# yangdongchao/RSTnet

Measured on NVIDIA H100. Metric: codec_frames_per_s, higher is better.
Workload: dtype f32

## Files before the change

### include/rstnet_b200.h

```cpp
#ifndef RSTNET_B200_H
#define RSTNET_B200_H

#include <stdint.h>

#ifdef __cplusplus
extern "C" {
#endif

typedef void* rstnet_stream_t;

enum { RSTNET_ACT_NONE = 0, RSTNET_ACT_ELU = 1, RSTNET_ACT_GELU = 2 };

int rstnet_version(void);
const char* rstnet_last_error(void);
int64_t rstnet_launch_count(void);
uint32_t rstnet_device_error_flags(int clear);

typedef struct {
  const float* A;
  int64_t a_batch_stride, a_row_stride;
  const float* Wt;
  const float* bias;
  const float* scale;
  const float* R;
  int64_t r_batch_stride, r_row_stride;
  float* C;
  int64_t c_batch_stride, c_row_stride;
  int32_t batch, rows, N, K;
  int32_t pre_act, post_act;
  int32_t taps;
  int64_t tap_stride;
} rstnet_gemm_rows_args;
int rstnet_gemm_rows_f32(const rstnet_gemm_rows_args* args, rstnet_stream_t stream);

typedef struct rstnet_tc_plan rstnet_tc_plan;
typedef struct {
  const float* A;
  int64_t a_i_stride, a_o_stride;
  int32_t a_c_extent, a_i_extent, a_o_extent;
  int32_t taps, tap_di, tap_do, o_mul;
  const float* W;
  const float* W_lo;
  int32_t N, Kc;
  int32_t I_out, O_out;
  float* C;
  int64_t c_i_stride, c_o_stride, c_split_stride;
  const float* R;
  int64_t r_i_stride, r_o_stride, r_split_stride;
  const float* bias;
  const float* scale;
  int32_t n_split;
  int32_t pre_act, post_act, precision;
  float* C2;
  int32_t act2;
} rstnet_tc_gemm_desc;
int rstnet_tc_gemm_create(const rstnet_tc_gemm_desc* desc, rstnet_tc_plan** out);
int rstnet_tc_gemm_run(const rstnet_tc_plan* plan, rstnet_stream_t stream);
void rstnet_tc_gemm_destroy(rstnet_tc_plan* plan);
int rstnet_tc_gemm_grid(const rstnet_tc_plan* plan, int32_t* grid_x, int32_t* grid_y, int32_t* tile_n);
int rstnet_tc_gemm_create_ex(const rstnet_tc_gemm_desc* desc, int32_t kpair, rstnet_tc_plan** out);
int rstnet_tc_gemm_kpair(const rstnet_tc_plan* plan, int32_t* on);
typedef struct rstnet_tc_resblock_plan rstnet_tc_resblock_plan;
typedef struct {
  const float* Y;
  int64_t y_i_stride, y_o_stride;
  int32_t channels;
  int32_t I_out, O_out, y_rows;
  const float* W1;
  const float* W1_lo;
  const float* b1;
  const float* W2;
  const float* W2_lo;
  const float* b2;
  float* out;
  int64_t out_i_stride, out_o_stride;
} rstnet_tc_resblock_desc;
int rstnet_tc_resblock_create(const rstnet_tc_resblock_desc* desc, rstnet_tc_resblock_plan** out);
int rstnet_tc_resblock_run(const rstnet_tc_resblock_plan* plan, rstnet_stream_t stream);
void rstnet_tc_resblock_destroy(rstnet_tc_resblock_plan* plan);

int rstnet_tf32_split_f32(const float* x, float* hi, float* lo, int64_t n, rstnet_stream_t stream);

int rstnet_conv1d_cin1_f32(const float* x, int64_t x_batch_stride, int64_t x_time_stride, const float* w, const float* bias,
                           float* out, float* out2 , int64_t out_batch_stride,
                           int64_t out_time_stride, int32_t batch, int32_t T, int32_t Cout, int32_t k,
                           int32_t post_act, int32_t act2, rstnet_stream_t stream);

int rstnet_conv1d_cout1_f32(const float* x, int64_t x_batch_stride, int64_t x_time_stride, const float* w,
                            const float* bias, float* out, int64_t out_batch_stride, int32_t batch,
                            int32_t T, int32_t Cin, int32_t k, rstnet_stream_t stream);

int rstnet_convtr1d_depthwise_f32(const float* x, int64_t x_batch_stride, int64_t x_time_stride,
                                  const float* w, float* out, int64_t out_batch_stride,
                                  int64_t out_time_stride, int32_t batch, int32_t T, int32_t C,
                                  int32_t stride, rstnet_stream_t stream);

int rstnet_rows_fill_f32(float* buf, int64_t batch_stride, int32_t batch, int32_t C, int32_t row0,
                         int32_t nrows, int32_t mode, int32_t src_row, const int64_t* only_if_zero,
                         int32_t only_if_zero_stride ,
                         int32_t channels_per_stream, rstnet_stream_t stream);
int rstnet_rows_fill_tail_f32(float* buf, int64_t batch_stride, int32_t batch, int32_t C, int32_t row0, int32_t nrows,
                              int32_t mode, const int64_t* valid, int64_t valid_div, int32_t channels_per_stream,
                              rstnet_stream_t stream);
typedef struct {
  float* buf;
  int64_t batch_stride;
  int32_t C, src_row, dst_row, nrows;
  int32_t cps;
  int32_t reserved;
} rstnet_row_copy;
int rstnet_rows_copy_table_f32(const rstnet_row_copy* table_dev, int32_t n_entries, int32_t batch,
                               const int64_t* active, rstnet_stream_t stream);
int rstnet_counter_add(int64_t* counter, int64_t delta, int32_t n, const int64_t* active ,
                       rstnet_stream_t stream);
int rstnet_counter_add_rows(int64_t* counter, const int64_t* delta, int32_t n, rstnet_stream_t stream);

int rstnet_layer_norm_f32(const float* x, int64_t x_batch_stride, const float* weight, const float* bias,
                          float* y, int32_t batch, int32_t rows_per_batch, int32_t dim, float eps,
                          rstnet_stream_t stream);

int rstnet_rope_kv_append_f32(float* qkv, int64_t q_batch_stride, int64_t q_time_stride, float* kv,
                              const int64_t* offset, int32_t offset_stride, const float* freqs, int32_t batch,
                              int32_t T, int32_t H, int32_t D, int32_t cap, rstnet_stream_t stream);
int rstnet_ring_attention_f32(const float* qkv, int64_t q_batch_stride, int64_t q_time_stride,
                              const float* kv, const int64_t* offset, int32_t offset_stride, float* out,
                              int64_t o_batch_stride, int64_t o_time_stride, int32_t batch, int32_t T,
                              int32_t H, int32_t D, int32_t cap, int32_t context, int32_t linear,
                              rstnet_stream_t stream);
int rstnet_rope_ring_attention_f32(const float* qkv, int64_t q_batch_stride, int64_t q_time_stride, float* kv,
                                   const int64_t* offset, int32_t offset_stride, const float* freqs, float* out,
                                   int64_t o_batch_stride, int64_t o_time_stride, int32_t batch, int32_t T, int32_t H,
                                   int32_t D, int32_t cap, int32_t context, rstnet_stream_t stream);

int64_t rstnet_rvq_encode_workspace(int64_t N, int32_t n_q, int32_t dim, int32_t bins);
int rstnet_rvq_encode_f32(const float* x, int64_t ldx, const float* E, const float* Et,
                          const float* enorm, int64_t* codes, void* work, int64_t N, int32_t T,
                          int32_t n_q, int32_t n_q_semantic, int32_t dim, int32_t bins,
                          int32_t time_major, rstnet_stream_t stream);
int rstnet_rvq_decode_gather_f32(const int64_t* codes, const float* E, float* q, int64_t N, int32_t T,
                                 int32_t n_q, int32_t n_q_semantic, int32_t dim, int32_t bins,
                                 int32_t time_major, rstnet_stream_t stream);

#define RSTNET_RESAMPLE_MAX_TABLE_BYTES (48 * 1024)
int rstnet_resample_f32(const float* x, int64_t x_row_stride, int64_t x_len, int64_t x_shift, const float* taps,
                        const int32_t* start, int32_t n, int32_t o, int32_t S, int32_t start_max, float* out,
                        int64_t out_row_stride, int64_t out_len, int32_t rows, rstnet_stream_t stream);

#define RSTNET_STFT_FRAMES_PER_BLOCK 16
int64_t rstnet_stft_loss_workspace(int32_t clips, int64_t max_len, int32_t hop);
int rstnet_stft_loss_sums_f32(const float* ref, const float* deg, const int64_t* offsets, const int64_t* lengths,
                              int32_t clips, int64_t min_len, int64_t max_len, int32_t n_fft, int32_t hop, int32_t win,
                              const float* twiddle, const float* window, double* sums, int32_t n_res, int32_t res,
                              void* ws, int64_t ws_bytes, rstnet_stream_t stream);

#define RSTNET_SISNR_SAMPLES_PER_BLOCK 8192
int64_t rstnet_sisnr_moments_workspace(int32_t clips, int64_t max_len);
int rstnet_sisnr_moments_f32(const float* ref, const float* deg, const int64_t* offsets, const int64_t* lengths,
                             int32_t clips, int64_t max_len, double* moments, void* ws, int64_t ws_bytes,
                             rstnet_stream_t stream);


typedef struct rstnet_skinny_plan rstnet_skinny_plan;
int64_t rstnet_skinny_gemm_workspace(int32_t M, int32_t N, int32_t max_splits);
int rstnet_skinny_gemm_create(const void* X, const void* W, const void* R, void* out, float* partial_ws,
                              int32_t M, int32_t N, int32_t K, int32_t max_splits, rstnet_skinny_plan** plan);
int rstnet_skinny_gemm_create_fused(const void* X, const void* W, const void* R, void* out, float* partial_ws,
                                    int32_t M, int32_t N, int32_t K, int32_t max_splits, int32_t fin_mode,
                                    const void* norm_w, void* aux_out, float eps, int32_t kyutai,
                                    rstnet_skinny_plan** plan);
int rstnet_skinny_gemm_run(const rstnet_skinny_plan* plan, rstnet_stream_t stream);
void rstnet_skinny_gemm_destroy(rstnet_skinny_plan* plan);

int rstnet_lm_embed_sum_bf16(const int64_t* seq, int32_t seq_stride, const void* wte, int64_t wte_rows,
                             const void* const* tables_dev, int64_t table_rows, int32_t n_q, int32_t E, void* x, int32_t rows,
                             rstnet_stream_t stream);
int rstnet_lm_embed_rows_bf16(const int64_t* ids, int32_t id_stride, const void* table, int64_t table_rows, int32_t D,
                              void* out, int32_t rows, rstnet_stream_t stream);
int rstnet_lm_rms_norm_bf16(const void* x, const void* w, void* y, int32_t rows, int32_t dim, float eps, int32_t kyutai,
                            rstnet_stream_t stream);
int rstnet_lm_rope_kv_append_bf16(const void* qkv, const void* cos_tab, const void* sin_tab, int64_t rope_rows, int32_t rope_n,
                                  const int64_t* offset, int32_t offset_stride ,
                                  const int32_t* row_stream, const int32_t* row_tl, void* q_out, void* kv, int32_t rows,
                                  int32_t B, int32_t n_head, int32_t n_kv, int32_t hs, int32_t cap, rstnet_stream_t stream);
#define RSTNET_KV_LOG2_PAGE_MIN 4
#define RSTNET_KV_LOG2_PAGE_MAX 12
int rstnet_lm_rope_kv_append_paged_bf16(const void* qkv, const void* cos_tab, const void* sin_tab, int64_t rope_rows,
                                        int32_t rope_n, const int64_t* offset, int32_t offset_stride, const int32_t* row_stream,
                                        const int32_t* row_tl, void* q_out, void* kv, int32_t rows, int32_t B, int32_t n_head,
                                        int32_t n_kv, int32_t hs, int32_t cap, const int32_t* page_table, int32_t pages_stride,
                                        int32_t log2_page, rstnet_stream_t stream);
int rstnet_lm_rope_pair_kv_append_bf16(const void* qkv, const int64_t* offset, int32_t offset_stride, void* q_out, void* kv,
                                       int32_t rows, int32_t B, int32_t H, int32_t hd, int32_t cap, const float* freqs,
                                       rstnet_stream_t stream);
int rstnet_lm_rope_pair_kv_append_paged_bf16(const void* qkv, const int64_t* offset, int32_t offset_stride, void* q_out, void* kv,
                                             int32_t rows, int32_t B, int32_t H, int32_t hd, int32_t cap, const float* freqs,
                                             const int32_t* page_table, int32_t pages_stride, int32_t log2_page,
                                             rstnet_stream_t stream);
int rstnet_lm_rope_pair_kv_append_rows_bf16(const void* qkv, const int64_t* offset, const int32_t* row_stream, const int32_t* row_tl,
                                            void* q_out, void* kv, int32_t rows, int32_t B, int32_t H, int32_t hd, int32_t cap,
                                            const float* freqs, rstnet_stream_t stream);
int rstnet_lm_ring_decode_attention_bf16(const void* q, const void* kv, const int64_t* offset, int32_t offset_stride,
                                         const int32_t* row_stream, const int32_t* row_tl, void* out, int32_t rows, int32_t B,
                                         int32_t n_head, int32_t n_kv, int32_t hs, int32_t cap, int32_t context,
                                         rstnet_stream_t stream);
int rstnet_lm_paged_decode_attention_bf16(const void* q, const void* kv, const int64_t* offset, int32_t offset_stride,
                                          const int32_t* row_stream, const int32_t* row_tl, void* out, int32_t rows, int32_t B,
                                          int32_t n_head, int32_t n_kv, int32_t hs, int32_t cap, int32_t context,
                                          const int32_t* page_table, int32_t pages_stride, int32_t log2_page,
                                          rstnet_stream_t stream);
int rstnet_lm_silu_mul_bf16(const void* ab, void* out, int32_t M, int32_t I, rstnet_stream_t stream);
int rstnet_lm_depth_attention_bf16(const void* qkv, void* kvd, void* out, int32_t B, int32_t H, int32_t hd, int32_t cap,
                                   int32_t step, int32_t ring_quirk, rstnet_stream_t stream);
int rstnet_lm_sample_params_bf16(const void* logits, int32_t rows, int32_t V, int32_t n_valid, const int32_t* n_valid_rows,
                                 int32_t n_valid_stride, int32_t top_k, float temp, float top_p, const int32_t* top_k_rows,
                                 const float* temp_rows, const float* top_p_rows, int32_t param_stride, uint32_t seed,
                                 const int64_t* step_counter, const int64_t* step_rows, const uint32_t* key_rows,
                                 int64_t* tokens, int32_t tok_stride, rstnet_stream_t stream);

int rstnet_lm_cross_entropy_bf16(const void* logits, int64_t row_stride, int32_t rows, int32_t V, int32_t groups,
                                 const int64_t* labels, const int64_t* ignore_ids, const float* weights,
                                 const int32_t* row_slot, int32_t n_slots, float* nll, int32_t* pred, double* acc,
                                 rstnet_stream_t stream);

int rstnet_lm_delay_cache_in(int64_t* cache, const int64_t* off, const int64_t* active, const int64_t* delays,
                             const int64_t* user, int32_t user_stride, int64_t* seq, int32_t seq_stride, int32_t B, int32_t K,
                             int32_t dep_q, int32_t CT, int64_t text_init, int64_t audio_init, rstnet_stream_t stream);
int rstnet_lm_delay_cache_out(int64_t* cache, int64_t* off, const int64_t* active, const int64_t* delays,
                              const int64_t* tokens, int32_t tok_stride, int64_t* out, int32_t out_stride, int64_t* valid,
                              int32_t B, int32_t K, int32_t dep_q, int32_t CT, int32_t max_delay, rstnet_stream_t stream);

typedef struct {
  void* base;
  int64_t stride_bytes;
  int64_t bytes;
  int32_t count;
  int64_t staging_offset;
} rstnet_segment;
int rstnet_segments_gather(const rstnet_segment* table_dev, int32_t n, void* staging, int32_t ctas, rstnet_stream_t s);
int rstnet_segments_scatter(const rstnet_segment* table_dev, int32_t n, const void* staging, int32_t ctas, rstnet_stream_t s);

#define RSTNET_KV_COPY_MAX_POOLS 256
int rstnet_kv_pages_copy(const void* const* pools, int32_t n_pools, const int32_t* pairs, int32_t n_pairs, int64_t page_bytes,
                         int32_t ctas, rstnet_stream_t s);

#define RSTNET_GEN_REC 5
enum { RSTNET_GEN_HELD = 0, RSTNET_GEN_FIXED = 1, RSTNET_GEN_WINDOWED = 2, RSTNET_GEN_ARGMAX = 4 };
enum { RSTNET_GEN_RUNNING = 0, RSTNET_GEN_LAST = 1, RSTNET_GEN_STOPPED = 2, RSTNET_GEN_IDLE = 3 };
int rstnet_lm_gen_rows_advance(const int64_t* tokens, int32_t tok_stride, int32_t* rec, int32_t* row_valid, int32_t valid_stride,
                               int32_t* status, int32_t B, int32_t dep_q, int32_t card, rstnet_stream_t stream);

#ifdef __cplusplus
}
#endif
#endif
```

### rstnet_b200/_lib.py

```python
from __future__ import annotations

import ctypes as C
import os

_HERE = os.path.dirname(os.path.abspath(__file__))
LIB_PATH = os.path.join(_HERE, "lib", "librstnet_b200.so")

ACT_NONE, ACT_ELU, ACT_GELU = 0, 1, 2

SYMBOLS = [
    "rstnet_version", "rstnet_last_error", "rstnet_launch_count", "rstnet_device_error_flags",
    "rstnet_gemm_rows_f32", "rstnet_tc_gemm_create", "rstnet_tc_gemm_run", "rstnet_tc_gemm_destroy", "rstnet_tc_gemm_grid",
    "rstnet_tc_gemm_create_ex", "rstnet_tc_gemm_kpair",
    "rstnet_tc_resblock_create", "rstnet_tc_resblock_run", "rstnet_tc_resblock_destroy", "rstnet_tf32_split_f32", "rstnet_conv1d_cin1_f32", "rstnet_conv1d_cout1_f32",
    "rstnet_convtr1d_depthwise_f32", "rstnet_rows_fill_f32", "rstnet_rows_copy_table_f32",
    "rstnet_counter_add", "rstnet_layer_norm_f32", "rstnet_rope_kv_append_f32",
    "rstnet_ring_attention_f32", "rstnet_rope_ring_attention_f32", "rstnet_rvq_encode_workspace", "rstnet_rvq_encode_f32",
    "rstnet_rvq_decode_gather_f32",
    "rstnet_skinny_gemm_workspace", "rstnet_skinny_gemm_create", "rstnet_skinny_gemm_create_fused", "rstnet_skinny_gemm_run", "rstnet_skinny_gemm_destroy",
    "rstnet_lm_embed_sum_bf16", "rstnet_lm_embed_rows_bf16", "rstnet_lm_rms_norm_bf16", "rstnet_lm_rope_kv_append_bf16",
    "rstnet_lm_rope_pair_kv_append_bf16",
    "rstnet_lm_ring_decode_attention_bf16", "rstnet_lm_silu_mul_bf16", "rstnet_lm_depth_attention_bf16",
    "rstnet_resample_f32", "rstnet_lm_delay_cache_in", "rstnet_lm_delay_cache_out", "rstnet_counter_add_rows",
    "rstnet_lm_cross_entropy_bf16", "rstnet_rows_fill_tail_f32", "rstnet_lm_sample_params_bf16",
    "rstnet_lm_rope_kv_append_paged_bf16", "rstnet_lm_paged_decode_attention_bf16", "rstnet_lm_rope_pair_kv_append_paged_bf16",
    "rstnet_stft_loss_workspace", "rstnet_stft_loss_sums_f32", "rstnet_sisnr_moments_workspace", "rstnet_sisnr_moments_f32",
    "rstnet_segments_gather", "rstnet_segments_scatter", "rstnet_lm_rope_pair_kv_append_rows_bf16",
    "rstnet_kv_pages_copy", "rstnet_lm_gen_rows_advance",
]

KV_LOG2_PAGE_MIN, KV_LOG2_PAGE_MAX = 4, 12
KV_COPY_MAX_POOLS = 256
GEN_REC = 5
GEN_HELD, GEN_FIXED, GEN_WINDOWED, GEN_ARGMAX = 0, 1, 2, 4
GEN_RUNNING, GEN_LAST, GEN_STOPPED, GEN_IDLE = 0, 1, 2, 3

RESAMPLE_MAX_TABLE_BYTES = 48 * 1024

STFT_FRAMES_PER_BLOCK = 16
SISNR_SAMPLES_PER_BLOCK = 8192


class GemmRowsArgs(C.Structure):
    _fields_ = [
        ("A", C.c_void_p), ("a_batch_stride", C.c_int64), ("a_row_stride", C.c_int64),
        ("Wt", C.c_void_p), ("bias", C.c_void_p), ("scale", C.c_void_p),
        ("R", C.c_void_p), ("r_batch_stride", C.c_int64), ("r_row_stride", C.c_int64),
        ("C", C.c_void_p), ("c_batch_stride", C.c_int64), ("c_row_stride", C.c_int64),
        ("batch", C.c_int32), ("rows", C.c_int32), ("N", C.c_int32), ("K", C.c_int32),
        ("pre_act", C.c_int32), ("post_act", C.c_int32), ("taps", C.c_int32), ("tap_stride", C.c_int64),
    ]


class TcGemmDesc(C.Structure):
    _fields_ = [
        ("A", C.c_void_p), ("a_i_stride", C.c_int64), ("a_o_stride", C.c_int64),
        ("a_c_extent", C.c_int32), ("a_i_extent", C.c_int32), ("a_o_extent", C.c_int32),
        ("taps", C.c_int32), ("tap_di", C.c_int32), ("tap_do", C.c_int32), ("o_mul", C.c_int32),
        ("W", C.c_void_p), ("W_lo", C.c_void_p), ("N", C.c_int32), ("Kc", C.c_int32), ("I_out", C.c_int32), ("O_out", C.c_int32),
        ("C", C.c_void_p), ("c_i_stride", C.c_int64), ("c_o_stride", C.c_int64), ("c_split_stride", C.c_int64),
        ("R", C.c_void_p), ("r_i_stride", C.c_int64), ("r_o_stride", C.c_int64), ("r_split_stride", C.c_int64),
        ("bias", C.c_void_p), ("scale", C.c_void_p),
        ("n_split", C.c_int32), ("pre_act", C.c_int32), ("post_act", C.c_int32), ("precision", C.c_int32),
        ("C2", C.c_void_p), ("act2", C.c_int32),
    ]


class TcResblockDesc(C.Structure):
    _fields_ = [
        ("Y", C.c_void_p), ("y_i_stride", C.c_int64), ("y_o_stride", C.c_int64),
        ("channels", C.c_int32), ("I_out", C.c_int32), ("O_out", C.c_int32), ("y_rows", C.c_int32),
        ("W1", C.c_void_p), ("W1_lo", C.c_void_p), ("b1", C.c_void_p),
        ("W2", C.c_void_p), ("W2_lo", C.c_void_p), ("b2", C.c_void_p),
        ("out", C.c_void_p), ("out_i_stride", C.c_int64), ("out_o_stride", C.c_int64),
    ]


class RowCopy(C.Structure):
    _fields_ = [("buf", C.c_void_p), ("batch_stride", C.c_int64), ("C", C.c_int32), ("src_row", C.c_int32),
                ("dst_row", C.c_int32), ("nrows", C.c_int32), ("cps", C.c_int32), ("reserved", C.c_int32)]


class Segment(C.Structure):
    _fields_ = [("base", C.c_void_p), ("stride_bytes", C.c_int64), ("bytes", C.c_int64), ("count", C.c_int32),
                ("staging_offset", C.c_int64)]


class RstnetError(RuntimeError):
    pass


_lib = None


def lib() -> C.CDLL:
    global _lib
    if _lib is not None:
        return _lib
    if not os.path.exists(LIB_PATH):
        raise RstnetError(
            f"{LIB_PATH} not found: the CUDA extension is not built. Run `python -m rstnet_b200.build` "
            "(there is no CPU fallback).")
    from . import build as _build
    stamp = os.path.join(os.path.dirname(LIB_PATH), "build.sha256")
    if os.path.isdir(_build.CSRC) and (not os.path.exists(stamp) or open(stamp).read().strip() != _build._digest()):
        raise RstnetError(
            f"{LIB_PATH} is stale (built from different sources than rstnet_b200/csrc + include/). "
            "Run `python -m rstnet_b200.build`.")
    L = C.CDLL(LIB_PATH)
    vp, i32, i64, f32 = C.c_void_p, C.c_int32, C.c_int64, C.c_float
    L.rstnet_version.restype = C.c_int
    L.rstnet_last_error.restype = C.c_char_p
    L.rstnet_launch_count.restype = i64
    L.rstnet_gemm_rows_f32.argtypes = [C.POINTER(GemmRowsArgs), vp]
    L.rstnet_tc_gemm_create.argtypes = [C.POINTER(TcGemmDesc), C.POINTER(C.c_void_p)]
    L.rstnet_tc_gemm_run.argtypes = [vp, vp]
    L.rstnet_tc_gemm_destroy.argtypes = [vp]
    L.rstnet_tc_gemm_destroy.restype = None
    L.rstnet_tc_gemm_grid.argtypes = [vp, C.POINTER(i32), C.POINTER(i32), C.POINTER(i32)]
    L.rstnet_tc_gemm_create_ex.argtypes = [C.POINTER(TcGemmDesc), i32, C.POINTER(C.c_void_p)]
    L.rstnet_tc_gemm_kpair.argtypes = [vp, C.POINTER(i32)]
    L.rstnet_tc_resblock_create.argtypes = [C.POINTER(TcResblockDesc), C.POINTER(C.c_void_p)]
    L.rstnet_tc_resblock_run.argtypes = [vp, vp]
    L.rstnet_tc_resblock_destroy.argtypes = [vp]
    L.rstnet_tc_resblock_destroy.restype = None
    L.rstnet_tf32_split_f32.argtypes = [vp, vp, vp, i64, vp]
    L.rstnet_conv1d_cin1_f32.argtypes = [vp, i64, i64, vp, vp, vp, vp, i64, i64, i32, i32, i32, i32, i32, i32, vp]
    L.rstnet_conv1d_cout1_f32.argtypes = [vp, i64, i64, vp, vp, vp, i64, i32, i32, i32, i32, vp]
    L.rstnet_convtr1d_depthwise_f32.argtypes = [vp, i64, i64, vp, vp, i64, i64, i32, i32, i32, i32, vp]
    L.rstnet_rows_fill_f32.argtypes = [vp, i64, i32, i32, i32, i32, i32, i32, vp, i32, i32, vp]
    L.rstnet_rows_fill_tail_f32.argtypes = [vp, i64, i32, i32, i32, i32, i32, vp, i64, i32, vp]
    L.rstnet_rows_copy_table_f32.argtypes = [vp, i32, i32, vp, vp]
    L.rstnet_counter_add.argtypes = [vp, i64, i32, vp, vp]
    L.rstnet_layer_norm_f32.argtypes = [vp, i64, vp, vp, vp, i32, i32, i32, f32, vp]
    L.rstnet_rope_kv_append_f32.argtypes = [vp, i64, i64, vp, vp, i32, vp, i32, i32, i32, i32, i32, vp]
    L.rstnet_ring_attention_f32.argtypes = [vp, i64, i64, vp, vp, i32, vp, i64, i64, i32, i32, i32, i32, i32, i32, i32, vp]
    L.rstnet_rope_ring_attention_f32.argtypes = [vp, i64, i64, vp, vp, i32, vp, vp, i64, i64, i32, i32, i32, i32, i32, i32, vp]
    L.rstnet_rvq_encode_workspace.argtypes = [i64, i32, i32, i32]
    L.rstnet_rvq_encode_workspace.restype = i64
    L.rstnet_rvq_encode_f32.argtypes = [vp, i64, vp, vp, vp, vp, vp, i64, i32, i32, i32, i32, i32, i32, vp]
    L.rstnet_rvq_decode_gather_f32.argtypes = [vp, vp, vp, i64, i32, i32, i32, i32, i32, i32, vp]
    L.rstnet_skinny_gemm_workspace.argtypes = [i32, i32, i32]
    L.rstnet_skinny_gemm_workspace.restype = i64
    L.rstnet_skinny_gemm_create.argtypes = [vp, vp, vp, vp, vp, i32, i32, i32, i32, C.POINTER(C.c_void_p)]
    L.rstnet_skinny_gemm_create_fused.argtypes = [vp, vp, vp, vp, vp, i32, i32, i32, i32, i32, vp, vp, f32, i32, C.POINTER(C.c_void_p)]
    L.rstnet_skinny_gemm_run.argtypes = [vp, vp]
    L.rstnet_skinny_gemm_destroy.argtypes = [vp]
    L.rstnet_skinny_gemm_destroy.restype = None
    L.rstnet_lm_embed_sum_bf16.argtypes = [vp, i32, vp, i64, vp, i64, i32, i32, vp, i32, vp]
    L.rstnet_lm_embed_rows_bf16.argtypes = [vp, i32, vp, i64, i32, vp, i32, vp]
    L.rstnet_device_error_flags.argtypes = [i32]
    L.rstnet_device_error_flags.restype = C.c_uint32
    L.rstnet_lm_rms_norm_bf16.argtypes = [vp, vp, vp, i32, i32, f32, i32, vp]
    L.rstnet_lm_rope_kv_append_bf16.argtypes = [vp, vp, vp, i64, i32, vp, i32, vp, vp, vp, vp, i32, i32, i32, i32, i32, i32, vp]
    L.rstnet_lm_rope_pair_kv_append_bf16.argtypes = [vp, vp, i32, vp, vp, i32, i32, i32, i32, i32, vp, vp]
    L.rstnet_lm_rope_pair_kv_append_paged_bf16.argtypes = [vp, vp, i32, vp, vp, i32, i32, i32, i32, i32, vp, vp, i32, i32, vp]
    L.rstnet_lm_rope_pair_kv_append_rows_bf16.argtypes = [vp, vp, vp, vp, vp, vp, i32, i32, i32, i32, i32, vp, vp]
    L.rstnet_lm_ring_decode_attention_bf16.argtypes = [vp, vp, vp, i32, vp, vp, vp, i32, i32, i32, i32, i32, i32, i32, vp]
    L.rstnet_lm_rope_kv_append_paged_bf16.argtypes = [vp, vp, vp, i64, i32, vp, i32, vp, vp, vp, vp, i32, i32, i32, i32, i32, i32,
                                                      vp, i32, i32, vp]
    L.rstnet_lm_paged_decode_attention_bf16.argtypes = [vp, vp, vp, i32, vp, vp, vp, i32, i32, i32, i32, i32, i32, i32, vp, i32, i32,
                                                        vp]
    L.rstnet_lm_silu_mul_bf16.argtypes = [vp, vp, i32, i32, vp]
    L.rstnet_lm_depth_attention_bf16.argtypes = [vp, vp, vp, i32, i32, i32, i32, i32, i32, vp]
    L.rstnet_resample_f32.argtypes = [vp, i64, i64, i64, vp, vp, i32, i32, i32, i32, vp, i64, i64, i32, vp]
    L.rstnet_lm_delay_cache_in.argtypes = [vp, vp, vp, vp, vp, i32, vp, i32, i32, i32, i32, i32, i64, i64, vp]
    L.rstnet_lm_delay_cache_out.argtypes = [vp, vp, vp, vp, vp, i32, vp, i32, vp, i32, i32, i32, i32, i32, vp]
    L.rstnet_counter_add_rows.argtypes = [vp, vp, i32, vp]
    L.rstnet_lm_cross_entropy_bf16.argtypes = [vp, i64, i32, i32, i32, vp, vp, vp, vp, i32, vp, vp, vp, vp]
    L.rstnet_lm_sample_params_bf16.argtypes = [vp, i32, i32, i32, vp, i32, i32, f32, f32, vp, vp, vp, i32, C.c_uint32, vp, vp, vp,
                                               vp, i32, vp]
    L.rstnet_stft_loss_workspace.argtypes = [i32, i64, i32]
    L.rstnet_stft_loss_workspace.restype = i64
    L.rstnet_stft_loss_sums_f32.argtypes = [vp, vp, vp, vp, i32, i64, i64, i32, i32, i32, vp, vp, vp, i32, i32, vp, i64, vp]
    L.rstnet_sisnr_moments_workspace.argtypes = [i32, i64]
    L.rstnet_sisnr_moments_workspace.restype = i64
    L.rstnet_sisnr_moments_f32.argtypes = [vp, vp, vp, vp, i32, i64, vp, vp, i64, vp]
    L.rstnet_segments_gather.argtypes = [vp, i32, vp, i32, vp]
    L.rstnet_segments_scatter.argtypes = [vp, i32, vp, i32, vp]
    L.rstnet_kv_pages_copy.argtypes = [vp, i32, vp, i32, i64, i32, vp]
    L.rstnet_lm_gen_rows_advance.argtypes = [vp, i32, vp, vp, i32, vp, i32, i32, i32, vp]
    for name in SYMBOLS:
        fn = getattr(L, name)
        if fn.restype is C.c_int and name not in ("rstnet_version",):
            pass
    _lib = L
    return L


def check(rc: int, what: str = "") -> None:
    if rc != 0:
        msg = lib().rstnet_last_error()
        raise RstnetError(f"{what or 'rstnet call'} failed (rc={rc}): {msg.decode() if msg else '?'}")


def launch_count() -> int:
    return int(lib().rstnet_launch_count())
```

### rstnet_b200/codec.py

```python
from __future__ import annotations

import math
from contextlib import contextmanager
from typing import Dict, Iterable, Iterator, List, Optional, Tuple

import numpy as np
import torch
from torch import nn

from . import ops
from ._lib import ACT_ELU, ACT_GELU, ACT_NONE, RstnetError
from .row_state import segs, tensor_segs


def on_own_device(fn):
    import functools

    @functools.wraps(fn)
    def wrapper(self, *a, **kw):
        dev = self.device
        if dev.type != "cuda" or torch.cuda.current_device() == (dev.index if dev.index is not None else torch.cuda.current_device()):
            return fn(self, *a, **kw)
        with torch.cuda.device(dev):
            return fn(self, *a, **kw)
    return wrapper


class _Node(nn.Module):
    """Anonymous container so that parameters get the reference's dotted state_dict names."""


def _register(root: nn.Module, dotted: str, tensor: torch.Tensor, buffer: bool = False) -> None:
    *path, leaf = dotted.split(".")
    m = root
    for p in path:
        if p not in m._modules:
            m.add_module(p, _Node())
        m = m._modules[p]
    if buffer:
        m.register_buffer(leaf, tensor)
    else:
        m.register_parameter(leaf, nn.Parameter(tensor, requires_grad=False))


_OLD_CODEBOOK_NAMES = {"inited": "_initialized", "cluster_size": "cluster_usage", "embed_avg": "embedding_sum",
                       "embed_sum": "embedding_sum"}


class MimiCodec(nn.Module):

    def __init__(self, sample_rate=24000, n_filters=64, encoder_rates=[4, 5, 6, 8], compress=2, causal=True,
                 latent_dim=512, codebook_size=4096, codebook_dim=32, rvq_layers=8, num_heads=8, num_layers=8,
                 layer_scale=0.01, context=250, dim_feedforward=2048, semantic_feature_dim=1024,
                 target_frame_rate=12.5):
        super().__init__()
        if not causal:
            raise NotImplementedError("only the causal codec (the streaming hot path) is implemented")
        self.sample_rate = sample_rate
        self.n_filters = n_filters
        self.ratios = list(encoder_rates)
        self.compress = compress
        self.latent_dim = latent_dim
        self.codebook_size, self.codebook_dim, self.n_q, self.n_q_semantic = codebook_size, codebook_dim, rvq_layers, 1
        self.num_heads, self.num_layers = num_heads, num_layers
        self.context, self.dim_feedforward = context, 2048
        self.max_period = 10000.0
        self.kernel_size, self.last_kernel_size, self.residual_kernel_size = 7, 3, 3
        self.hop_length = int(math.prod(self.ratios))
        self.encoder_frame_rate = sample_rate / self.hop_length
        self.target_frame_rate = target_frame_rate
        self.resample_stride = int(self.encoder_frame_rate / self.target_frame_rate)
        self.frame_size = self.hop_length * self.resample_stride
        self.codebook_eps = 1e-5
        assert latent_dim % num_heads == 0 and n_filters % (4 * compress) == 0 and codebook_dim % 16 == 0

        D, nf = latent_dim, n_filters
        g = torch.Generator().manual_seed(0)

        def w_(shape):
            t = torch.empty(shape)
            if len(shape) >= 2:
                nn.init.xavier_uniform_(t, generator=g)
            else:
                t.zero_()
            return t

        def conv(prefix, cout, cin, k, bias=True):
            _register(self, f"{prefix}.weight", w_((cout, cin, k)))
            if bias:
                _register(self, f"{prefix}.bias", w_((cout,)))

        def resblock(prefix, dim):
            conv(f"{prefix}.block.1.conv.conv", dim // compress, dim, self.residual_kernel_size)
            conv(f"{prefix}.block.3.conv.conv", dim, dim // compress, 1)

        idx, mult = 0, 1
        conv(f"encoder.model.{idx}.conv.conv", nf, 1, self.kernel_size)
        idx += 1
        for r in reversed(self.ratios):
            resblock(f"encoder.model.{idx}", mult * nf)
            idx += 2
            conv(f"encoder.model.{idx}.conv.conv", mult * nf * 2, mult * nf, 2 * r)
            idx += 1
            mult *= 2
        idx += 1
        conv(f"encoder.model.{idx}.conv.conv", D, mult * nf, self.last_kernel_size)
        idx, mult = 0, 2 ** len(self.ratios)
        conv(f"decoder.model.{idx}.conv.conv", mult * nf, D, self.kernel_size)
        idx += 1
        for r in self.ratios:
            idx += 1
            _register(self, f"decoder.model.{idx}.convtr.convtr.weight", w_((mult * nf, mult * nf // 2, 2 * r)))
            _register(self, f"decoder.model.{idx}.convtr.convtr.bias", w_((mult * nf // 2,)))
            idx += 1
            resblock(f"decoder.model.{idx}", mult * nf // 2)
            idx += 1
            mult //= 2
        idx += 1
        conv(f"decoder.model.{idx}.conv.conv", 1, nf, self.last_kernel_size)
        s = self.resample_stride
        _register(self, "downsample.conv.conv.conv.weight", w_((D, D, 2 * s)))
        _register(self, "upsample.convtr.convtr.convtr.weight", w_((D, 1, 2 * s)))
        _register(self, "semantic_mapping_layer.ln_layer.weight", w_((D, semantic_feature_dim)))
        _register(self, "semantic_mapping_layer.ln_layer.bias", w_((D,)))
        for side in ("encoder_transformer", "decoder_transformer"):
            for l in range(num_layers):
                p = f"{side}.transformer.layers.{l}"
                _register(self, f"{p}.self_attn.in_proj_weight", w_((3 * D, D)))
                _register(self, f"{p}.self_attn.out_proj.weight", w_((D, D)))
                for n in ("norm1", "norm2"):
                    _register(self, f"{p}.{n}.weight", torch.ones(D))
                    _register(self, f"{p}.{n}.bias", torch.zeros(D))
                _register(self, f"{p}.linear1.weight", w_((self.dim_feedforward, D)))
                _register(self, f"{p}.linear2.weight", w_((D, self.dim_feedforward)))
                _register(self, f"{p}.layer_scale_1.scale", torch.full((D,), float(layer_scale)))
                _register(self, f"{p}.layer_scale_2.scale", torch.full((D,), float(layer_scale)))
        for part, n in (("rvq_first", self.n_q_semantic), ("rvq_rest", self.n_q - self.n_q_semantic)):
            _register(self, f"quantizer.{part}.input_proj.weight", w_((codebook_dim, D, 1)))
            _register(self, f"quantizer.{part}.output_proj.weight", w_((D, codebook_dim, 1)))
            for i in range(n):
                p = f"quantizer.{part}.vq.layers.{i}._codebook"
                _register(self, f"{p}._initialized", torch.tensor([False], dtype=torch.float), buffer=True)
                _register(self, f"{p}.cluster_usage", torch.ones(codebook_size), buffer=True)
                _register(self, f"{p}.embedding_sum", torch.zeros(codebook_size, codebook_dim), buffer=True)
        self._engine: Optional["_Engine"] = None
        self._stream_state: Optional["_StreamState"] = None
        self.use_cuda_graphs = True
        self.streaming_tensor_cores = True
        self.tc_precision = 0
        self.decoder_precision = 0
        self.resblock_tensor_cores = True
        self.batch_tensor_cores_min = 96
        self.fused_rope_attention = True
        self.fused_resblock = True
        self.elu_in_transform_max_channels = 0

    def load_state_dict(self, state_dict, strict: bool = True, **kw):
        sd = {}
        for k, v in state_dict.items():
            head, _, leaf = k.rpartition(".")
            if head.endswith("_codebook") and leaf in _OLD_CODEBOOK_NAMES:
                k = f"{head}.{_OLD_CODEBOOK_NAMES[leaf]}"
            sd[k] = v
        self._engine = None
        return super().load_state_dict(sd, strict=strict, **kw)

    def _apply(self, fn, *a, **kw):
        self._engine = None
        return super()._apply(fn, *a, **kw)

    @classmethod
    def from_config(cls, config_path):
        import json
        with open(config_path, "r") as f:
            return cls(**json.load(f))

    @property
    def device(self) -> torch.device:
        return next(self.parameters()).device

    def _eng(self) -> "_Engine":
        dev = self.device
        if dev.type != "cuda":
            raise RstnetError("MimiCodec runs on CUDA only (sm_90a kernels; the CPU path is the reference itself)")
        if self._engine is None or self._engine.device != dev:
            self._engine = _Engine(self, dev)
        return self._engine

    @torch.no_grad()
    @on_own_device
    def encode(self, audio_data: torch.Tensor) -> torch.Tensor:
        if audio_data.dim() != 3 or audio_data.shape[1] != 1:
            raise ValueError(f"expected audio of shape [B,1,L], got {tuple(audio_data.shape)}")
        eng = self._eng()
        x = audio_data.to(device=eng.device, dtype=torch.float32)
        if self._stream_state is not None:
            return self._stream_state.encode(x)
        return eng.encode_batch(x)

    @torch.no_grad()
    @on_own_device
    def decode(self, codes: torch.Tensor) -> torch.Tensor:
        if codes.dim() != 3:
            raise ValueError(f"expected codes of shape [B,K,T], got {tuple(codes.shape)}")
        if codes.dtype.is_floating_point:
            raise ValueError("codes must be integers")
        eng = self._eng()
        c = codes.to(device=eng.device, dtype=torch.int64).contiguous()
        if self._stream_state is not None:
            return self._stream_state.decode(c)
        return eng.decode_batch(c)

    def encode_many(self, items: Iterable[Tuple[object, torch.Tensor]], capacity: int = 128) -> Iterator[Tuple[object, torch.Tensor]]:
        return _corpus_run(self._eng(), items, int(capacity), "enc", CORPUS_CHUNK_FRAMES)

    def decode_many(self, items: Iterable[Tuple[object, torch.Tensor]], capacity: int = 128) -> Iterator[Tuple[object, torch.Tensor]]:
        return _corpus_run(self._eng(), items, int(capacity), "dec", CORPUS_CHUNK_FRAMES)

    def forward(self, *a, **kw):
        raise NotImplementedError("training forward (with semantic distillation) is out of scope; use encode/decode")

    @property
    def is_streaming(self) -> bool:
        return self._stream_state is not None

    @on_own_device
    def streaming_forever(self, batch_size: int, clip_window: bool = False):
        self._stream_state = _StreamState(self._eng(), batch_size, clip_window)

    @contextmanager
    def streaming(self, batch_size: int, clip_window: bool = False):
        self.streaming_forever(batch_size, clip_window)
        try:
            yield
        finally:
            self._stream_state = None

    @on_own_device
    def reset_streaming(self, streams=None):
        if self._stream_state is None:
            raise ValueError("Trying to reset streaming, but the codec wasn't streaming.")
        self._stream_state.reset(streams)

    def set_active_streams(self, mask) -> None:
        if self._stream_state is None:
            raise ValueError("the codec is not streaming")
        self._stream_state.set_active(mask)

    def get_streaming_state(self):
        return {"": self._stream_state}

    def set_streaming_state(self, state):
        state = dict(state)
        if "" not in state:
            raise RuntimeError("Expected to find a streaming state for .")
        st = state.pop("")
        if state:
            raise RuntimeError(f"Some states were not consumed: {list(state.keys())}")
        if st is not None and (not isinstance(st, _StreamState) or st.eng is not self._eng()):
            raise RuntimeError("the streaming state belongs to another codec (or to weights that were since reloaded / moved)")
        self._stream_state = st


class MimiTokenizer:

    def __init__(self, model: MimiCodec, device=torch.device("cuda")):
        self.model = model.to(device).eval()
        self.device = device
        self.sr = 24000

    def find_length(self, x):
        return x.shape[1]

    def tokenize(self, wav, sample_rate: int = 24000):
        if not isinstance(wav, torch.Tensor):
            raise NotImplementedError
        if wav.dim() == 1:
            return wav
        if wav.dim() == 2:
            if wav.numel() == 0:
                return None
            if sample_rate != self.sr:
                raise NotImplementedError("resample to 24 kHz before tokenizing")
            wav = wav.unsqueeze(1)
        codes = self.model.encode(wav.to(self.device))
        return codes.squeeze(0).detach().cpu().to(torch.int16)

    def detokenize(self, codes):
        assert codes.shape[0] == 8
        wav = self.model.decode(codes.unsqueeze(0).to(self.device).long())
        return wav.squeeze(1).detach().cpu()


class MimiCodecBTK(MimiCodec):

    def encode(self, audio_data: torch.Tensor) -> torch.Tensor:
        return super().encode(audio_data).transpose(1, 2).contiguous()

    def decode(self, codes: torch.Tensor) -> torch.Tensor:
        if codes.dim() != 3:
            raise RstnetError(f"codes must be [B, T, K], got {tuple(codes.shape)}")
        return super().decode(codes.transpose(1, 2).contiguous())


class _Buf:

    def __init__(self, B: int, ctx: int, T: int, extra: int, C: int, device, tbc: bool):
        self.B, self.ctx, self.T, self.extra, self.C, self.tbc = B, ctx, T, extra, C, tbc
        self.rows = ctx + T + extra
        if tbc:
            self.t = torch.zeros(self.rows, B, C, device=device, dtype=torch.float32)
            self.ts, self.bs = B * C, C
        else:
            self.t = torch.zeros(B, self.rows, C, device=device, dtype=torch.float32)
            self.ts, self.bs = C, self.rows * C

    def off(self, row: int) -> int:
        return row * self.ts

    def zero_ctx(self, streams=None):
        if self.ctx:
            if streams is None:
                (self.t[:self.ctx] if self.tbc else self.t[:, :self.ctx]).zero_()
            elif self.tbc:
                self.t[:self.ctx, streams] = 0.0
            else:
                self.t[streams, :self.ctx] = 0.0

    def row_segments(self, b: int) -> np.ndarray:
        if not self.ctx:
            return segs()
        e = self.t.element_size()
        if self.tbc:
            return segs((self.t.data_ptr() + b * self.bs * e, self.ts * e, self.C * e, self.ctx))
        n = self.ctx * self.C * e
        return segs((self.t.data_ptr() + b * self.bs * e, n, n, 1))

    def carry_entry(self):
        if self.tbc:
            return (self.t, 0, self.B * self.C, self.T, 0, self.ctx, self.C)
        return (self.t, self.bs, self.C, self.T, 0, self.ctx, self.C)


class _Engine:

    BATCH_MODE_BYTES = 12 << 30

    def __init__(self, m: "MimiCodec", device: torch.device):
        self.m, self.device = m, device
        sd = {k: v.detach().to(device=device, dtype=torch.float32) for k, v in m.state_dict().items()}
        self.D, self.nf = m.latent_dim, m.n_filters
        self.ratios = list(m.ratios)
        self.enc_ratios = list(reversed(m.ratios))
        D = self.D

        def conv_w(prefix):
            w = sd[f"{prefix}.weight"]
            cout, cin, k = w.shape
            wk = w.permute(0, 2, 1).reshape(cout, k * cin).contiguous()
            return dict(W=wk, Wt=wk.t().contiguous(), bias=sd.get(f"{prefix}.bias"), taps=k)

        def convtr_w(prefix, s):
            w = sd[f"{prefix}.weight"]
            cin, cout, k = w.shape
            assert k == 2 * s
            w_prev = w[:, :, s:].permute(2, 1, 0).reshape(s * cout, cin)
            w_cur = w[:, :, :s].permute(2, 1, 0).reshape(s * cout, cin)
            wk = torch.cat([w_prev, w_cur], 1).contiguous()
            return dict(W=wk, Wt=wk.t().contiguous(), bias=sd[f"{prefix}.bias"].repeat(s).contiguous(), taps=2)

        def lin_w(w):
            w = w.contiguous()
            return dict(W=w, Wt=w.t().contiguous(), bias=None, taps=1)

        self.e_conv0_w = sd["encoder.model.0.conv.conv.weight"].reshape(self.nf, -1).contiguous()
        self.e_conv0_b = sd["encoder.model.0.conv.conv.bias"]
        self.e_res, self.e_down = [], []
        idx = 1
        for r in self.enc_ratios:
            self.e_res.append((conv_w(f"encoder.model.{idx}.block.1.conv.conv"), conv_w(f"encoder.model.{idx}.block.3.conv.conv")))
            idx += 2
            self.e_down.append(conv_w(f"encoder.model.{idx}.conv.conv"))
            idx += 1
        idx += 1
        self.e_final = conv_w(f"encoder.model.{idx}.conv.conv")
        self.down_w = conv_w("downsample.conv.conv.conv")
        self.d_conv0 = conv_w("decoder.model.0.conv.conv")
        self.d_tr, self.d_res = [], []
        idx = 1
        for r in self.ratios:
            idx += 1
            self.d_tr.append(convtr_w(f"decoder.model.{idx}.convtr.convtr", r))
            idx += 1
            self.d_res.append((conv_w(f"decoder.model.{idx}.block.1.conv.conv"), conv_w(f"decoder.model.{idx}.block.3.conv.conv")))
            idx += 1
        idx += 1
        wf = sd[f"decoder.model.{idx}.conv.conv.weight"]
        self.d_final_w = wf[0].t().contiguous().reshape(-1)
        self.d_final_b = sd[f"decoder.model.{idx}.conv.conv.bias"]
        self.up_w = sd["upsample.convtr.convtr.convtr.weight"].reshape(D, -1).contiguous()
        self.tr = {}
        for side in ("encoder_transformer", "decoder_transformer"):
            layers = []
            for l in range(m.num_layers):
                p = f"{side}.transformer.layers.{l}"
                layers.append(dict(
                    in_w=lin_w(sd[f"{p}.self_attn.in_proj_weight"]), out_w=lin_w(sd[f"{p}.self_attn.out_proj.weight"]),
                    n1w=sd[f"{p}.norm1.weight"], n1b=sd[f"{p}.norm1.bias"],
                    n2w=sd[f"{p}.norm2.weight"], n2b=sd[f"{p}.norm2.bias"],
                    w1=lin_w(sd[f"{p}.linear1.weight"]), w2=lin_w(sd[f"{p}.linear2.weight"]),
                    ls1=sd[f"{p}.layer_scale_1.scale"], ls2=sd[f"{p}.layer_scale_2.scale"]))
            self.tr[side] = layers
        hd = D // m.num_heads
        ds = torch.arange(hd // 2, dtype=torch.float32)
        self.freqs = torch.exp(ds * (-math.log(m.max_period) * 2 / hd)).to(device)
        cd = m.codebook_dim
        w1 = sd["quantizer.rvq_first.input_proj.weight"].reshape(cd, D)
        w2 = sd["quantizer.rvq_rest.input_proj.weight"].reshape(cd, D)
        self.q_in = lin_w(torch.cat([w1, w2], 0))
        o1 = sd["quantizer.rvq_first.output_proj.weight"].reshape(D, cd)
        o2 = sd["quantizer.rvq_rest.output_proj.weight"].reshape(D, cd)
        self.q_out = lin_w(torch.cat([o1, o2], 1))
        prefixes = [f"quantizer.rvq_first.vq.layers.{i}._codebook" for i in range(m.n_q_semantic)]
        prefixes += [f"quantizer.rvq_rest.vq.layers.{i}._codebook" for i in range(m.n_q - m.n_q_semantic)]
        embs = [sd[f"{p}.embedding_sum"].cpu() / sd[f"{p}.cluster_usage"].cpu().clamp(min=m.codebook_eps)[:, None] for p in prefixes]
        E = torch.stack(embs)
        self.E = E.contiguous().to(device)
        self.Et = E.transpose(1, 2).contiguous().to(device)
        self.enorm = E.pow(2).sum(dim=-1).contiguous().to(device)
        self.zero_counter = torch.zeros(1, dtype=torch.int64, device=device)
        self._plans: Dict[tuple, object] = {}

    def enc_plan(self, B: int, L: int) -> "_EncPlan":
        tc = B >= self.m.batch_tensor_cores_min
        key = ("enc", B, L, tc)
        if key not in self._plans:
            for k in [k for k in self._plans if k[0] == "enc"]:
                del self._plans[k]
            self._plans[key] = _EncPlan(self, B, L, streaming=False, tensor_cores=tc)
        return self._plans[key]

    def dec_plan(self, B: int, T: int) -> "_DecPlan":
        tc = B >= self.m.batch_tensor_cores_min
        key = ("dec", B, T, tc)
        if key not in self._plans:
            for k in [k for k in self._plans if k[0] == "dec"]:
                del self._plans[k]
            self._plans[key] = _DecPlan(self, B, T, streaming=False, tensor_cores=tc)
        return self._plans[key]

    def encode_batch(self, x: torch.Tensor) -> torch.Tensor:
        B, _, L = x.shape
        m = self.m
        if L == 0:
            return torch.empty((B, m.n_q, 0), dtype=torch.int64, device=self.device)
        per_stream = 4 * L * (self.nf * 3.6) + (1 << 20)
        sub = max(1, min(B, int(self.BATCH_MODE_BYTES // per_stream)))
        outs = []
        for b0 in range(0, B, sub):
            xb = x[b0:b0 + sub]
            outs.append(self.enc_plan(xb.shape[0], L).run(xb, None).clone())
        return outs[0] if len(outs) == 1 else torch.cat(outs, 0)

    def decode_batch(self, codes: torch.Tensor) -> torch.Tensor:
        B, K, T = codes.shape
        m = self.m
        if T == 0:
            return torch.empty((B, 1, 0), dtype=torch.float32, device=self.device)
        per_stream = 4 * T * m.frame_size * (self.nf * 3.6) + (1 << 20)
        sub = max(1, min(B, int(self.BATCH_MODE_BYTES // per_stream)))
        outs = []
        for b0 in range(0, B, sub):
            cb = codes[b0:b0 + sub].contiguous()
            outs.append(self.dec_plan(cb.shape[0], T).run(cb, None).clone())
        return outs[0] if len(outs) == 1 else torch.cat(outs, 0)


def _ceil_div(a: int, b: int) -> int:
    return -(-a // b)


class _Plan:

    def __init__(self, eng: _Engine, B: int, streaming: bool, tensor_cores: bool, active: Optional[torch.Tensor] = None,
                 corpus: bool = False):
        self.eng, self.B, self.streaming, self.tc = eng, B, streaming, tensor_cores
        self.active = active
        self.corpus = corpus
        self.ops_list = []
        self.graph: Optional[torch.cuda.CUDAGraph] = None
        self.precision = eng.m.decoder_precision if isinstance(self, _DecPlan) else eng.m.tc_precision

    def buf(self, ctx, T, extra, C) -> _Buf:
        return _Buf(self.B, ctx, T, extra, C, self.eng.device, self.tc)

    def elu_in_transform(self, C: int) -> bool:
        return self.tc and C <= self.eng.m.elu_in_transform_max_channels and self.precision == 0 and self.eng.m.resblock_tensor_cores

    def fused_resblock(self, C: int) -> bool:
        return (self.tc and C in (64, 128) and self.precision == 0 and self.eng.m.resblock_tensor_cores
                and self.eng.m.fused_resblock)

    def raw_resblock_input(self, C: int) -> bool:
        return not self.tc or self.elu_in_transform(C) or self.fused_resblock(C)

    def resblock(self, y: _Buf, ya: _Buf, h: Optional[_Buf], w1, w2, out: _Buf, T: int):
        if self.fused_resblock(y.C):
            assert ya is y and y.ctx == 2 and self.tc
            B = self.B
            w1_hi, w1_lo = self.tc_weights(w1)
            w2_hi, w2_lo = self.tc_weights(w2)
            plan = ops.TcResblock(y.t, 0, y.C, B * y.C, y.rows, B, T, w1_hi, w1_lo, w1["bias"], w2_hi, w2_lo, w2["bias"],
                                  out.t, out.off(out.ctx), out.C, B * out.C)
            self.add(plan.run)
            return
        self.conv(ya, 0, 1, w1, h, 0, T, pre=ACT_ELU if ya is y else ACT_NONE, post=ACT_ELU, ffma=self.tc)
        self.conv(h, 0, 1, w2, out, out.ctx, T, post=ACT_ELU, R=y, r_row0=y.ctx, ffma=self.tc)

    @staticmethod
    def tc_weights(pack):
        if "W_hi" not in pack:
            pack["W_hi"], pack["W_lo"] = ops.tf32_split(pack["W"])
        return pack["W_hi"], pack["W_lo"]

    def add(self, fn):
        self.ops_list.append(fn)

    def launch(self):
        for fn in self.ops_list:
            fn()

    def conv(self, A: _Buf, a_row0: int, stride: int, pack, out: _Buf, out_row0: int, T_out: int, *, pre=ACT_NONE,
             post=ACT_NONE, R: Optional[_Buf] = None, r_row0: int = 0, tr_stride: int = 0, out2: Optional[_Buf] = None,
             out2_row0: int = 0, ffma: bool = False):
        B, Cin = self.B, A.C
        taps = pack["taps"]
        N = pack["W"].shape[0]
        if not self.tc:
            kw = dict(bias=pack["bias"], pre_act=pre, post_act=post)
            if R is not None:
                kw.update(R=R.t, r_off=R.off(r_row0), r_bs=R.bs, r_rs=R.ts)
            self.add(lambda: ops.gemm_rows(A.t, A.off(a_row0), A.bs, stride * Cin, pack["Wt"], out.t, out.off(out_row0),
                                           out.bs, N, B, T_out, **kw))
            return
        if ffma and (Cin % 32 != 0 or self.precision != 0 or not self.eng.m.resblock_tensor_cores):
            assert not tr_stride and out2 is None
            kw = dict(bias=pack["bias"], pre_act=pre, post_act=post, taps=taps, tap_stride=B * Cin)
            if R is not None:
                kw.update(R=R.t, r_off=R.off(r_row0), r_bs=B * R.C, r_rs=R.C)
            self.add(lambda: ops.gemm_rows(A.t, A.off(a_row0), stride * B * Cin, Cin, pack["Wt"], out.t, out.off(out_row0),
                                           B * out.C, out.C, T_out, B, **kw))
            return
        kw = dict(taps=taps, tap_do=1, o_mul=stride, bias=pack["bias"], pre_act=pre, post_act=post, precision=self.precision)
        if R is not None:
            kw.update(R=R.t, r_off=R.off(r_row0), r_i_stride=R.C, r_o_stride=B * R.C)
        if tr_stride:
            kw.update(n_split=out.C, c_split_stride=B * out.C)
        if out2 is not None:
            kw.update(C2=out2.t, c2_off=out2.off(out2_row0), act2=ACT_ELU)
        w_hi, w_lo = self.tc_weights(pack)
        plan = ops.TcGemm(A.t, A.off(a_row0), Cin, B * Cin, Cin, B, A.rows - a_row0, w_hi, Cin, out.t, out.off(out_row0),
                          out.C, (tr_stride or 1) * B * out.C, B, T_out, W_lo=w_lo, **kw)
        self.add(plan.run)

    def linear(self, A_t, a_rows_view, K, pack, out_t, out_view, N_row_stride, *, post=ACT_NONE, scale=None, R_view=None):
        a_off, nb, rpb, a_bs = a_rows_view
        c_off, _, _, c_bs = out_view
        if not self.tc:
            kw = dict(post_act=post, scale=scale)
            if R_view is not None:
                kw.update(R=out_t, r_off=R_view[0], r_bs=R_view[3], r_rs=N_row_stride)
            self.add(lambda: ops.gemm_rows(A_t, a_off, a_bs, K, pack["Wt"], out_t, c_off, c_bs, N_row_stride, nb, rpb, **kw))
            return
        assert nb == 1
        kw = dict(post_act=post, scale=scale, precision=self.precision)
        if R_view is not None:
            kw.update(R=out_t, r_off=R_view[0], r_i_stride=N_row_stride, r_o_stride=rpb * N_row_stride)
        w_hi, w_lo = self.tc_weights(pack)
        plan = ops.TcGemm(A_t, a_off, K, rpb * K, K, rpb, 1, w_hi, K, out_t, c_off, N_row_stride, rpb * N_row_stride, rpb, 1,
                          W_lo=w_lo, **kw)
        self.add(plan.run)

    def rows_view(self, X: _Buf, row0: int, nrows: int):
        if self.tc:
            return (X.off(row0), 1, nrows * self.B, 0)
        return (X.off(row0), self.B, nrows, X.bs)

    def flat_view(self, nrows: int, width: int):
        if self.tc:
            return (0, 1, nrows * self.B, 0)
        return (0, self.B, nrows, nrows * width)

    def ring_cap(self, F: int) -> int:
        if not self.streaming:
            return F
        return self.eng.m.context + (F if self.corpus else 0)

    def transformer(self, side: str, X: _Buf, x_row: int, F: int, cap: int):
        eng, m, B = self.eng, self.eng.m, self.B
        D, H, FF = eng.D, m.num_heads, m.dim_feedforward
        hd = D // H
        dev = eng.device
        ln = torch.empty(B * F, D, device=dev)
        qkv = torch.empty(B * F, 3 * D, device=dev)
        att = torch.empty(B * F, D, device=dev)
        ff = torch.empty(B * F, FF, device=dev)
        self.scratch = (ln, qkv, att, ff)
        if self.streaming:
            kv = [torch.zeros(2, B, H, cap, hd, device=dev) for _ in range(m.num_layers)]
            offset = torch.zeros(B, dtype=torch.int64, device=dev)
        else:
            kv = [torch.zeros(2, B, H, cap, hd, device=dev)] * m.num_layers
            offset = eng.zero_counter
        self.kv, self.offset, self.cap = kv, offset, cap
        xv = self.rows_view(X, x_row, F)
        if self.tc:
            q_bs, q_ts, o_bs, o_ts = 3 * D, B * 3 * D, D, B * D
            ln_args = (1, F * B)
        else:
            q_bs, q_ts, o_bs, o_ts = F * 3 * D, 3 * D, F * D, D
            ln_args = (B, F)
        x_bs = 0 if self.tc else X.bs
        linear = not self.streaming
        for l, w in enumerate(eng.tr[side]):
            kvl = kv[l]
            self.add(lambda w=w: ops.layer_norm(X.t, xv[0], x_bs, w["n1w"], w["n1b"], ln, ln_args[0], ln_args[1], D, 1e-5))
            self.linear(ln, self.flat_view(F, D), D, w["in_w"], qkv, self.flat_view(F, 3 * D), 3 * D)
            if self.streaming and F == 2 and hd == 64 and m.fused_rope_attention and min(q_bs, q_ts, o_bs, o_ts) % 4 == 0:
                self.add(lambda kvl=kvl: ops.rope_ring_attention(qkv, q_bs, q_ts, kvl, offset, eng.freqs, att, o_bs, o_ts, B, F, H, hd,
                                                                 cap, m.context))
            else:
                self.add(lambda kvl=kvl: ops.rope_kv_append(qkv, q_bs, q_ts, kvl, offset, eng.freqs, B, F, H, hd, cap))
                self.add(lambda kvl=kvl: ops.ring_attention(qkv, q_bs, q_ts, kvl, offset, att, o_bs, o_ts, B, F, H, hd, cap, m.context,
                                                            linear))
            self.linear(att, self.flat_view(F, D), D, w["out_w"], X.t, xv, D, scale=w["ls1"], R_view=xv)
            self.add(lambda w=w: ops.layer_norm(X.t, xv[0], x_bs, w["n2w"], w["n2b"], ln, ln_args[0], ln_args[1], D, 1e-5))
            self.linear(ln, self.flat_view(F, D), D, w["w1"], ff, self.flat_view(F, FF), FF, post=ACT_GELU)
            self.linear(ff, self.flat_view(F, FF), FF, w["w2"], X.t, xv, D, scale=w["ls2"], R_view=xv)

    def finish_streaming(self, carries: List[_Buf], F: int):
        if not self.streaming:
            return
        dev = self.eng.device
        self.carries = carries
        entries = [b.carry_entry() for b in carries if b.ctx]
        table = ops.make_copy_table(entries, dev)
        n, nb = len(entries), (1 if self.tc else self.B)
        self.copy_table = table
        self.add(lambda: ops.rows_copy_table(table, n, nb, self.active))
        self.add(lambda: ops.counter_add(self.offset, F, self.active))

    def row_segments(self, b: int):
        regions = [(f"carry{i}", buf.row_segments(b)) for i, buf in enumerate(self.carries) if buf.ctx]
        for l, kv in enumerate(self.kv):
            e = kv.element_size()
            regions.append((f"ring{l}", segs((kv[0, b].data_ptr(), kv.stride(0) * e, kv[0, b].numel() * e, 2))))
        regions.append(("offset", tensor_segs(self.offset[b:b + 1])))
        return regions

    def reset(self, streams=None):
        assert self.streaming
        for b in self.carries:
            b.zero_ctx(streams)
        if streams is None:
            self.offset.zero_()
        else:
            self.offset[streams] = 0


class _EncPlan(_Plan):

    def __init__(self, eng: _Engine, B: int, L: int, streaming: bool, tensor_cores: bool, active: Optional[torch.Tensor] = None,
                 valid: Optional[torch.Tensor] = None):
        super().__init__(eng, B, streaming, tensor_cores, active, corpus=valid is not None)
        m, dev = eng.m, eng.device
        self.L = L
        if streaming and L % m.frame_size != 0:
            raise RstnetError(f"streaming chunks must be multiples of {m.frame_size} samples, got {L}")
        nf, D = eng.nf, eng.D
        k0 = m.kernel_size
        T = [L]
        for r in eng.enc_ratios:
            T.append(_ceil_div(T[-1], r))
        self.F = F = T[-1]
        s = m.resample_stride
        self.T5 = T5 = _ceil_div(F, s)
        self.xin = xin = self.buf(k0 - 1, L, 0, 1)
        y, ya, h, r_ = [], [], [], []
        C = nf
        for i, ratio in enumerate(eng.enc_ratios):
            own_copy = not self.raw_resblock_input(C)
            y.append(self.buf(0 if own_copy else m.residual_kernel_size - 1, T[i], 0, C))
            ya.append(self.buf(m.residual_kernel_size - 1, T[i], 0, C) if own_copy else y[-1])
            h.append(None if self.fused_resblock(C) else self.buf(0, T[i], 0, C // m.compress))
            r_.append(self.buf(ratio, T[i], T[i + 1] * ratio - T[i], C))
            C *= 2
        y4 = self.buf(m.last_kernel_size - 1, F, 0, C)
        X = self.buf(s, F, T5 * s - F, D)
        cd = m.codebook_dim
        self.lat = lat = torch.empty(B * T5, D, device=dev)
        xproj = torch.empty(B * T5, 2 * cd, device=dev)
        self.codes = codes = torch.zeros(B, m.n_q, T5, dtype=torch.int64, device=dev)
        work = torch.empty(ops.rvq_encode_workspace(B * T5, m.n_q, cd, m.codebook_size), dtype=torch.uint8, device=dev)
        self._keep = (xproj, work)

        if self.tc and ya[0] is not y[0]:
            self.add(lambda: ops.conv1d_cin1(xin.t, xin.bs, xin.ts, eng.e_conv0_w, eng.e_conv0_b, y[0].t, 0, y[0].bs, y[0].ts, B, L,
                                             nf, k0, ACT_NONE, out2=ya[0].t, out2_off=ya[0].off(ya[0].ctx), act2=ACT_ELU))
        else:
            self.add(lambda: ops.conv1d_cin1(xin.t, xin.bs, xin.ts, eng.e_conv0_w, eng.e_conv0_b, y[0].t, y[0].off(y[0].ctx),
                                             y[0].bs, y[0].ts, B, L, nf, k0, ACT_NONE))
        for i, ratio in enumerate(eng.enc_ratios):
            w1, w2 = eng.e_res[i]
            self.resblock(y[i], ya[i], h[i], w1, w2, r_[i], T[i])
            if valid is not None:
                self.tail_fill(r_[i], T[i], 0, valid, math.prod(eng.enc_ratios[:i]))
            if i + 1 < len(y):
                nxt = y[i + 1]
                self.conv(r_[i], 0, ratio, eng.e_down[i], nxt, nxt.ctx, T[i + 1],
                          out2=ya[i + 1] if ya[i + 1] is not nxt else None, out2_row0=ya[i + 1].ctx)
            else:
                self.conv(r_[i], 0, ratio, eng.e_down[i], y4, y4.ctx, T[i + 1], post=ACT_ELU)
        self.conv(y4, 0, 1, eng.e_final, X, X.ctx, F)
        self.transformer("encoder_transformer", X, X.ctx, F, self.ring_cap(F))
        fill_bs, fill_nb, fill_C = (0, 1, B * D) if self.tc else (X.bs, B, D)
        only0 = self.offset if streaming else None
        self.add(lambda: ops.rows_fill(X.t, fill_bs, fill_nb, fill_C, 0, X.ctx, mode=1, src_row=X.ctx, only_if_zero=only0,
                                       channels_per_stream=D))
        if X.extra:
            self.add(lambda: ops.rows_fill(X.t, fill_bs, fill_nb, fill_C, X.ctx + X.T, X.extra, mode=1, src_row=X.ctx + X.T - 1))
        if valid is not None:
            self.tail_fill(X, F, 1, valid, eng.m.hop_length)
        lat_buf = _LatView(lat, B, T5, D, self.tc)
        self.conv(X, 0, s, eng.down_w, lat_buf, 0, T5)
        self.linear(lat, self.flat_view(T5, D), D, eng.q_in, xproj, self.flat_view(T5, 2 * cd), 2 * cd)
        self.add(lambda: ops.rvq_encode(xproj, 2 * cd, eng.E, eng.Et, eng.enorm, codes, work, B * T5, T5, m.n_q, m.n_q_semantic,
                                        cd, m.codebook_size, time_major=self.tc))
        self.finish_streaming([xin] + ya + r_ + [y4, X], F)

    def tail_fill(self, X: _Buf, T: int, mode: int, valid: torch.Tensor, div: int):
        bs, nb, C = (0, 1, self.B * X.C) if self.tc else (X.bs, self.B, X.C)
        self.add(lambda: ops.rows_fill_tail(X.t, bs, nb, C, X.ctx, T, mode, valid, div, channels_per_stream=X.C))

    def run(self, x: torch.Tensor, graphs: Optional[bool]) -> torch.Tensor:
        xin, L = self.xin, self.L
        if self.tc:
            xin.t[xin.ctx:xin.ctx + L, :, 0].copy_(x[:, 0, :].t())
        else:
            xin.t[:, xin.ctx:xin.ctx + L, 0].copy_(x[:, 0, :])
        _run_plan(self, graphs)
        return self.codes


class _LatView:

    def __init__(self, t: torch.Tensor, B: int, T: int, C: int, tbc: bool):
        self.t, self.C, self.ctx, self.rows, self.tbc = t, C, 0, T, tbc
        self.ts, self.bs = (B * C, C) if tbc else (C, T * C)

    def off(self, row: int) -> int:
        return row * self.ts


class _DecPlan(_Plan):

    def __init__(self, eng: _Engine, B: int, T: int, streaming: bool, tensor_cores: bool, n_codes: Optional[int] = None,
                 active: Optional[torch.Tensor] = None, corpus: bool = False):
        super().__init__(eng, B, streaming, tensor_cores, active, corpus)
        m, dev = eng.m, eng.device
        self.T = T
        D, nf = eng.D, eng.nf
        s = m.resample_stride
        self.F = F = T * s
        cd = m.codebook_dim
        K = n_codes or m.n_q
        self.codes_in = codes_in = torch.zeros(B, K, T, dtype=torch.int64, device=dev)
        q = torch.empty(B * T, 2 * cd, device=dev)
        qup = self.buf(1, T, 0, D)
        X = self.buf(m.kernel_size - 1, F, 0, D)
        C = nf * 2 ** len(eng.ratios)
        a = [self.buf(1, F, 0, C)]
        yd, yda, hd_ = [], [], []
        Tin = F
        for i, r in enumerate(eng.ratios):
            Tout = Tin * r
            own_copy = not self.raw_resblock_input(C // 2)
            yd.append(self.buf(0 if own_copy else m.residual_kernel_size - 1, Tout, 0, C // 2))
            yda.append(self.buf(m.residual_kernel_size - 1, Tout, 0, C // 2) if own_copy else yd[-1])
            hd_.append(None if self.fused_resblock(C // 2) else self.buf(0, Tout, 0, C // 2 // m.compress))
            last = i == len(eng.ratios) - 1
            a.append(self.buf((m.last_kernel_size - 1) if last else 1, Tout, 0, C // 2))
            C //= 2
            Tin = Tout
        self.Lout = Lout = Tin
        self.wav = wav = torch.empty(B, 1, Lout, device=dev)

        self.add(lambda: ops.rvq_decode_gather(codes_in, eng.E, q, B * T, T, K, m.n_q_semantic, cd, m.codebook_size,
                                               time_major=self.tc))
        self.linear(q, self.flat_view(T, 2 * cd), 2 * cd, eng.q_out, qup.t, self.rows_view(qup, 1, T), D)
        self.add(lambda: ops.convtr1d_depthwise(qup.t, qup.bs, qup.ts, eng.up_w, X.t, X.off(X.ctx), X.bs, X.ts, B, T, D, s))
        self.transformer("decoder_transformer", X, X.ctx, F, self.ring_cap(F))
        self.conv(X, 0, 1, eng.d_conv0, a[0], 1, F, post=ACT_ELU)
        Tin = F
        for i, r in enumerate(eng.ratios):
            self.conv(a[i], 0, 1, eng.d_tr[i], yd[i], yd[i].ctx, Tin, tr_stride=r, out2=yda[i] if yda[i] is not yd[i] else None,
                      out2_row0=yda[i].ctx)
            Tout = Tin * r
            w1, w2 = eng.d_res[i]
            self.resblock(yd[i], yda[i], hd_[i], w1, w2, a[i + 1], Tout)
            Tin = Tout
        last = a[-1]
        self.add(lambda: ops.conv1d_cout1(last.t, last.bs, last.ts, eng.d_final_w, eng.d_final_b, wav, Lout, B, Lout, last.C,
                                          m.last_kernel_size))
        self.finish_streaming([qup, X] + a + yda, F)
        self.debug_bufs = {"qup": [qup], "X": [X], "a": a, "yd": yd, "yda": yda, "hd": [b for b in hd_ if b is not None]}

    def run(self, codes: torch.Tensor, graphs: Optional[bool]) -> torch.Tensor:
        self.codes_in.copy_(codes)
        _run_plan(self, graphs)
        return self.wav


def _run_plan(plan, graphs: Optional[bool]) -> None:
    if not graphs:
        plan.launch()
        return
    if plan.graph is None:
        plan.warmups = getattr(plan, "warmups", 0) + 1
        if plan.warmups <= 2:
            plan.launch()
            return
        torch.cuda.synchronize()
        plan.graph = ops.capture(plan.launch)
    plan.graph.replay()


class _StreamState:

    def __init__(self, eng: _Engine, batch_size: int, clip_window: bool = False):
        self.eng, self.B, self.clip_window = eng, batch_size, clip_window
        self.enc: Dict[int, _EncPlan] = {}
        self.dec: Dict[int, _DecPlan] = {}
        self.active = torch.ones(batch_size, dtype=torch.int64, device=eng.device)

    def encode(self, x: torch.Tensor) -> torch.Tensor:
        B, _, L = x.shape
        if B != self.B:
            raise RstnetError(f"streaming batch size is {self.B}, got {B}")
        if L == 0:
            return torch.empty((B, self.eng.m.n_q, 0), dtype=torch.int64, device=self.eng.device)
        return self._enc_plan(L).run(x, self.eng.m.use_cuda_graphs).clone()

    def _enc_plan(self, L: int) -> "_EncPlan":
        if L not in self.enc:
            if self.enc:
                raise RstnetError("the chunk size must stay constant within one streaming scope")
            self.enc[L] = _EncPlan(self.eng, self.B, L, True, self.eng.m.streaming_tensor_cores, active=self.active)
        return self.enc[L]

    def _dec_plan(self, T: int, K: int) -> "_DecPlan":
        if T not in self.dec:
            if self.dec:
                raise RstnetError("the chunk size must stay constant within one streaming scope")
            self.dec[T] = _DecPlan(self.eng, self.B, T, True, self.eng.m.streaming_tensor_cores, n_codes=K, active=self.active,
                                   corpus=self.clip_window)
        return self.dec[T]

    def row_segments(self, b: int, chunk: int, frames: int, n_codes: int):
        enc, dec = self._enc_plan(chunk), self._dec_plan(frames, n_codes)
        return [("enc." + n, s) for n, s in enc.row_segments(b)] + [("dec." + n, s) for n, s in dec.row_segments(b)]

    def decode(self, codes: torch.Tensor) -> torch.Tensor:
        B, K, T = codes.shape
        if B != self.B:
            raise RstnetError(f"streaming batch size is {self.B}, got {B}")
        return self._dec_plan(T, K).run(codes, self.eng.m.use_cuda_graphs).clone()

    def set_active(self, mask):
        if mask is None:
            self.active.fill_(1)
        else:
            self.active.copy_(torch.as_tensor(mask).to(device=self.eng.device, dtype=torch.int64).reshape(self.B))

    def reset(self, streams=None):
        if streams is not None:
            streams = torch.as_tensor(streams, dtype=torch.int64).reshape(-1)
            if streams.numel() and (int(streams.min()) < 0 or int(streams.max()) >= self.B):
                raise RstnetError(f"stream index outside [0, {self.B})")
            streams = streams.to(self.eng.device)
        for p in list(self.enc.values()) + list(self.dec.values()):
            p.reset(streams)


CORPUS_CHUNK_FRAMES = 8


class _CorpusScope:

    def __init__(self, eng: _Engine, B: int, kind: str, frames: int):
        m, dev = eng.m, eng.device
        self.eng, self.B, self.kind = eng, B, kind
        self.enc = kind == "enc"
        self.chunk = frames * m.frame_size if self.enc else frames
        self.hdr = 3 * 8 * B
        pay_shape = (B, 1, self.chunk) if self.enc else (B, m.n_q, frames)
        pay_dtype = torch.float32 if self.enc else torch.int64
        nbytes = self.hdr + math.prod(pay_shape) * pay_dtype.itemsize
        self.stage = torch.zeros(nbytes, dtype=torch.uint8, device=dev)
        self.host = [torch.zeros(nbytes, dtype=torch.uint8).pin_memory() for _ in range(2)]
        valid, active, self.reset_rows = (self.stage[i * 8 * B:(i + 1) * 8 * B].view(torch.int64) for i in range(3))
        self.payload = self.stage[self.hdr:].view(pay_dtype).view(pay_shape)
        tc = m.streaming_tensor_cores
        if self.enc:
            self.plan = _EncPlan(eng, B, self.chunk, True, tc, active=active, valid=valid)
            out = self.plan.codes
        else:
            self.plan = _DecPlan(eng, B, frames, True, tc, active=active, corpus=True)
            out = self.plan.wav
        self.out = [torch.empty(out.shape, dtype=out.dtype).pin_memory() for _ in range(2)]
        self.events = [torch.cuda.Event() for _ in range(2)]

    def host_views(self, k: int):
        h = self.host[k].numpy()
        B = self.B
        valid, active, reset = (h[i * 8 * B:(i + 1) * 8 * B].view(np.int64) for i in range(3))
        return valid, active, reset, h[self.hdr:].view(np.float32 if self.enc else np.int64).reshape(self.payload.shape)

    def submit(self, k: int, n_reset: int):
        self.stage.copy_(self.host[k], non_blocking=True)
        if n_reset:
            self.plan.reset(self.reset_rows[:n_reset])
        out = self.plan.run(self.payload, self.eng.m.use_cuda_graphs)
        self.out[k].copy_(out, non_blocking=True)
        self.events[k].record()


class _Clip:
    __slots__ = ("key", "data", "n", "pos", "parts", "done", "total")

    def __init__(self, key, data: np.ndarray, n: int, total: int):
        self.key, self.data, self.n, self.total = key, data, n, total
        self.pos, self.done, self.parts = 0, 0, []


@torch.no_grad()
def _corpus_run(eng: _Engine, items, B: int, kind: str, frames: int):
    if B < 1:
        raise ValueError(f"capacity must be at least 1, got {B}")
    m = eng.m
    enc = kind == "enc"
    fs = m.frame_size
    with torch.cuda.device(eng.device):
        scope = _CorpusScope(eng, B, kind, frames)
    chunk = scope.chunk
    source = iter(items)
    ready = []

    def next_clip() -> Optional[_Clip]:
        for key, x in source:
            if enc:
                w = torch.as_tensor(x).detach()
                if w.dim() != 1:
                    raise ValueError(f"encode_many: clip {key!r} must be a 1-D waveform [L], got {tuple(w.shape)}")
                w = np.ascontiguousarray(w.to("cpu", torch.float32).numpy())
                c = _Clip(key, w, w.shape[0], _ceil_div(w.shape[0], fs))
            else:
                cd = torch.as_tensor(x).detach()
                if cd.dim() != 2 or cd.shape[0] != m.n_q or cd.dtype.is_floating_point:
                    raise ValueError(f"decode_many: codes of {key!r} must be integers [{m.n_q}, T], got {cd.dtype} {tuple(cd.shape)}")
                cd = np.ascontiguousarray(cd.to("cpu", torch.int64).numpy())
                c = _Clip(key, cd, cd.shape[1], cd.shape[1] * fs)
            if c.n:
                return c
            ready.append((key, torch.empty((m.n_q, 0), dtype=torch.int64) if enc else torch.empty(0)))
        return None

    def harvest(k: int, records):
        scope.events[k].synchronize()
        out = scope.out[k].numpy()
        for b, c, ncols in records:
            c.parts.append(out[b, :, :ncols].copy() if enc else out[b, 0, :ncols].copy())
            c.done += ncols
            if c.done == c.total:
                ready.append((c.key, torch.from_numpy(np.concatenate(c.parts, -1))))

    rows: List[Optional[_Clip]] = [None] * B
    exhausted, pending, k = False, None, 0
    while True:
        valid, active, reset, pay = scope.host_views(k)
        n_reset, records = 0, []
        for b in range(B):
            c = rows[b]
            if c is not None and c.pos >= c.n:
                c = rows[b] = None
            if c is None and not exhausted:
                c = rows[b] = next_clip()
                if c is None:
                    exhausted = True
                else:
                    reset[n_reset] = b
                    n_reset += 1
            if c is None:
                valid[b], active[b] = chunk, 0
                continue
            take = min(chunk, c.n - c.pos)
            if enc:
                pay[b, 0, :take] = c.data[c.pos:c.pos + take]
                pay[b, 0, take:] = 0.0
                records.append((b, c, _ceil_div(take, fs)))
            else:
                pay[b, :, :take] = c.data[:, c.pos:c.pos + take]
                pay[b, :, take:] = 0
                records.append((b, c, take * fs))
            valid[b], active[b] = take, 1
            c.pos += take
        if records:
            with torch.cuda.device(eng.device):
                scope.submit(k, n_reset)
        if pending is not None:
            harvest(*pending)
        yield from ready
        ready.clear()
        if not records:
            return
        pending, k = (k, records), k ^ 1
```

### rstnet_b200/csrc/gemm_tc.cu

```cuda
#include <cstdlib>

#include "common.cuh"
#include "tc_common.cuh"
#include "../../include/rstnet_b200.h"

namespace rstnet {
extern void count_launch();
using namespace tc;

constexpr int TC_BM = 128;
constexpr int TC_BKE = 32;
constexpr int TC_A_BYTES = TC_BM * 128;
constexpr int TC_CONSUMER_WARPS = 8;
constexpr int TC_THREADS = 32 * TC_CONSUMER_WARPS + 32;
constexpr int TC_CHUNK_STAGES = 4;

struct TcParams {
  float* C;
  float* C2;
  int act2;
  long long c_i_stride, c_o_stride, c_split_stride;
  const float* R;
  long long r_i_stride, r_o_stride, r_split_stride;
  const float* bias;
  const float* scale;
  int n_split;
  int I_out, O_out, N, Kc;
  int taps, tap_di, tap_do, o_mul, kchunks;
  int pre_act, post_act, i_tiles;
  int m_tiles, n_tiles;
  int kpair;
};

template <int BN, int PREC>
struct TcCfg {
  static constexpr bool SPLIT = PREC == 0;
  static constexpr int B_BYTES = BN * 128;
  static constexpr int STAGE_BYTES = TC_A_BYTES + B_BYTES * (SPLIT ? 2 : 1);
  static constexpr int STAGES = (200 * 1024 / STAGE_BYTES) > 8 ? 8 : (200 * 1024 / STAGE_BYTES);
  static constexpr int SMEM_BYTES = STAGES * STAGE_BYTES + 1024  + 256 ;
  static constexpr int Q_PIECES = BN / 32;
  static_assert(STAGES % 2 == 0 && 2 * Q_PIECES <= STAGES, "K-pair rings and queue");
};

__device__ __forceinline__ float tf32_rna(float x) {
  const uint32_t u = __float_as_uint(x);
  return __uint_as_float((x != x ? u | 0x00400000u : u + 0x1000u) & 0xFFFFE000u);
}
__device__ __forceinline__ float tf32_rna_lo(float x, float hi) {
  const float d = x - hi;
  return d != d ? 0.f : __uint_as_float((__float_as_uint(d) + 0x1000u) & 0xFFFFE000u);
}

__device__ __forceinline__ float act_tc(float x, int act) {
  if (act == ACT_ELU) return elu_fast(x);
  if (act == ACT_GELU) return gelu_f(x);
  return x;
}

template <bool SPLIT, bool PRE_ELU>
__device__ __forceinline__ void tc_build_a(uint32_t st, uint32_t a_row, uint32_t a_sw, uint32_t (&ah)[4][4], uint32_t (&al)[4][4]) {
#pragma unroll
  for (int k = 0; k < 4; ++k) {
#pragma unroll
    for (int e = 0; e < 4; ++e) {
      const uint32_t chunk = (uint32_t)(2 * k + (e >> 1));
      float v;
      asm volatile("ld.shared.f32 %0, [%1];" : "=f"(v) : "r"(st + a_row + (e & 1) * 1024u + ((chunk ^ a_sw) << 4)));
      if (PRE_ELU) {
        const float e = __expf(v) - 1.f;
        v = v > 0.f ? v : e;
      }
      if (SPLIT) {
        const bool nonfinite = !(fabsf(v) < INFINITY);
        const float h = nonfinite ? 0.f : __uint_as_float((__float_as_uint(v) + 0x1000u) & 0xFFFFE000u);
        const float d = v - h;
        ah[k][e] = __float_as_uint(h);
        al[k][e] = (__float_as_uint(d) + (nonfinite ? 0u : 0x1000u)) & 0xFFFFE000u;
      } else {
        ah[k][e] = __float_as_uint(tf32_rna(v));
      }
    }
  }
}

template <int BN, bool SPLIT>
__device__ __forceinline__ void tc_mma_stage(float (&d0)[BN / 2], float (&d1)[BN / 2], const uint32_t (&ah)[4][4],
                                             const uint32_t (&al)[4][4], uint64_t db, uint64_t dbl, bool first) {
#pragma unroll
  for (int k = 0; k < 4; ++k) {
    const uint32_t acc_in = (first && k == 0) ? 0u : 1u;
    wgmma_tf32_rs<BN>(d0, ah[k], db + (uint64_t)(2 * k), acc_in);
    if (SPLIT) {
      wgmma_tf32_rs<BN>(d1, al[k], db + (uint64_t)(2 * k), acc_in);
      wgmma_tf32_rs<BN>(d1, ah[k], dbl + (uint64_t)(2 * k), 1u);
    }
  }
}

template <int BN, int PREC, bool PRE_ELU, bool KP>
__global__ void __launch_bounds__(TC_THREADS, 1)
gemm_tc_kernel(const __grid_constant__ CUtensorMap tmA, const __grid_constant__ CUtensorMap tmW,
               const __grid_constant__ CUtensorMap tmWlo, const TcParams p) {
  using Cfg = TcCfg<BN, PREC>;
  constexpr int S = Cfg::STAGES;
  constexpr int CH = TC_CHUNK_STAGES;
  constexpr int NR = BN / 2;
  extern __shared__ uint8_t smem_raw[];
  uint8_t* smem = smem_raw + ((1024u - (smem_u32(smem_raw) & 1023u)) & 1023u);
  uint64_t* full = reinterpret_cast<uint64_t*>(smem + S * Cfg::STAGE_BYTES);
  uint64_t* empty = full + S;
  uint64_t* qfull = empty + S;
  uint64_t* qempty = qfull + 2;
  const int warp = threadIdx.x / 32, lane = threadIdx.x % 32;
  const int total_k = p.taps * p.kchunks;
  const int total_tiles = p.m_tiles * p.n_tiles;
  const int bm = KP ? TC_BM / 2 : TC_BM;
  const int R = KP ? S / 2 : S;

  if (threadIdx.x == 0) {
    for (int s = 0; s < S; ++s) {
      mbar_init(&full[s], 1);
      mbar_init(&empty[s], KP ? TC_CONSUMER_WARPS / 2 : TC_CONSUMER_WARPS);
    }
    for (int q = 0; q < 2; ++q) {
      mbar_init(&qfull[q], 128);
      mbar_init(&qempty[q], 128);
    }
    fence_barrier_init();
  }
  __syncthreads();

  if (warp == TC_CONSUMER_WARPS) {
    if (elect_one()) {
      tma_prefetch_desc(&tmA);
      tma_prefetch_desc(&tmW);
      if (Cfg::SPLIT) tma_prefetch_desc(&tmWlo);
      int pos0 = 0, ph0 = 0, pos1 = 0, ph1 = 0;
      for (int t = blockIdx.x; t < total_tiles; t += gridDim.x) {
        const int nt = t % p.n_tiles, mt = t / p.n_tiles;
        const int i0 = (mt % p.i_tiles) * bm, ot = mt / p.i_tiles, n0 = nt * BN;
        for (int kit = 0; kit < total_k; ++kit) {
          const int w = KP ? (kit / TC_CHUNK_STAGES) & 1 : 0;
          const int pos = w ? pos1 : pos0, ph = w ? ph1 : ph0;
          const int s = w * R + pos;
          const int npos = pos + 1 == R ? 0 : pos + 1, nph = ph ^ (npos == 0);
          if (w) { pos1 = npos; ph1 = nph; } else { pos0 = npos; ph0 = nph; }
          mbar_wait(&empty[s], ph ^ 1);
          const int tap = kit / p.kchunks, kc = kit % p.kchunks;
          uint8_t* st = smem + s * Cfg::STAGE_BYTES;
          mbar_arrive_expect_tx(&full[s], Cfg::STAGE_BYTES - (TC_BM - bm) * 128);
          tma_load_3d(st, &tmA, &full[s], kc * TC_BKE, i0 + tap * p.tap_di, ot * p.o_mul + tap * p.tap_do);
          tma_load_2d(st + TC_A_BYTES, &tmW, &full[s], kit * TC_BKE, n0);
          if (Cfg::SPLIT) tma_load_2d(st + TC_A_BYTES + Cfg::B_BYTES, &tmWlo, &full[s], kit * TC_BKE, n0);
        }
      }
    }
    return;
  }

  const int wg = warp / 4, wq = warp % 4, gq = lane / 4, tq = lane % 4;
  const int r0 = (KP ? 0 : wg * 64) + wq * 16 + gq;
  const uint32_t a_row = (uint32_t)r0 * 128u + (uint32_t)tq * 4u, a_sw = (uint32_t)(r0 & 7);
  const uint32_t smem0 = smem_u32(smem);
  float acc[NR], d0[NR], d1[NR];
#pragma unroll
  for (int j = 0; j < NR; ++j) d0[j] = d1[j] = 0.f;
  const int nch = (total_k + CH - 1) / CH;
  const bool sender = KP && wg == 1;
  auto qel = [&](int q, int j) {
    return reinterpret_cast<float*>(smem + (q * Cfg::Q_PIECES + j / 16) * Cfg::STAGE_BYTES + TC_A_BYTES / 2) +
           (j % 16) * 128 + (threadIdx.x & 127);
  };
  int qn = 0;
  auto take_queued = [&]() {
    mbar_wait(&qfull[qn & 1], (qn >> 1) & 1);
#pragma unroll
    for (int j = 0; j < NR; ++j) acc[j] += *qel(qn & 1, j);
    mbar_arrive(&qempty[qn & 1]);
    ++qn;
  };
  const int base = KP ? wg * R : 0;
  int pos = 0, ph = 0;
  for (int t = blockIdx.x; t < total_tiles; t += gridDim.x) {
    const int nt = t % p.n_tiles, mt = t / p.n_tiles;
    const int i0 = (mt % p.i_tiles) * bm, ot = mt / p.i_tiles, n0 = nt * BN;
#pragma unroll
    for (int j = 0; j < NR; ++j) acc[j] = 0.f;
    for (int c = KP ? wg : 0; c < nch; c += KP ? 2 : 1) {
      const int k0 = c * CH;
      const int nst = total_k - k0 < CH ? total_k - k0 : CH;
      for (int u = 0; u < nst; ++u) {
        const int s = base + pos;
        mbar_wait(&full[s], ph);
        const uint32_t st = smem0 + (uint32_t)(s * Cfg::STAGE_BYTES);
        uint32_t ah[4][4], al[4][4];
        tc_build_a<Cfg::SPLIT, PRE_ELU>(st, a_row, a_sw, ah, al);
        const uint64_t db = gmma_desc_sw128(st + TC_A_BYTES);
        const uint64_t dbl = gmma_desc_sw128(st + TC_A_BYTES + Cfg::B_BYTES);
        wgmma_fence();
        tc_mma_stage<BN, Cfg::SPLIT>(d0, d1, ah, al, db, dbl, u == 0);
        wgmma_commit();
        wgmma_wait<0>();
        __syncwarp();
        if (lane == 0) mbar_arrive(&empty[s]);
        pos = pos + 1 == R ? 0 : pos + 1;
        ph ^= pos == 0;
      }
      fence_acc(d0);
      if (Cfg::SPLIT) fence_acc(d1);
      if (sender) {
        mbar_wait(&qempty[qn & 1], ((qn >> 1) & 1) ^ 1);
#pragma unroll
        for (int j = 0; j < NR; ++j) *qel(qn & 1, j) = Cfg::SPLIT ? d0[j] + d1[j] : d0[j];
        mbar_arrive(&qfull[qn & 1]);
        ++qn;
      } else {
        if (KP && c > 0) take_queued();
#pragma unroll
        for (int j = 0; j < NR; ++j) acc[j] += Cfg::SPLIT ? d0[j] + d1[j] : d0[j];
      }
    }
    if (KP && !sender && nch % 2 == 0) take_queued();
    if (sender) continue;
#pragma unroll
    for (int h = 0; h < 2; ++h) {
      const int i = i0 + r0 + 8 * h;
      if (i >= p.I_out) continue;
      float* crow = p.C + (long long)ot * p.c_o_stride + (long long)i * p.c_i_stride;
      float* crow2 = p.C2 ? p.C2 + (long long)ot * p.c_o_stride + (long long)i * p.c_i_stride : nullptr;
      const float* rrow = p.R ? p.R + (long long)ot * p.r_o_stride + (long long)i * p.r_i_stride : nullptr;
#pragma unroll
      for (int b = 0; b < BN / 8; ++b) {
        const int n = n0 + 8 * b + 2 * tq;
        if (n < p.N) {
          float2 v = make_float2(acc[4 * b + 2 * h], acc[4 * b + 2 * h + 1]);
          if (p.bias) {
            const float2 bb = *reinterpret_cast<const float2*>(p.bias + n);
            v.x += bb.x; v.y += bb.y;
          }
          if (p.scale) {
            const float2 ss = *reinterpret_cast<const float2*>(p.scale + n);
            v.x *= ss.x; v.y *= ss.y;
          }
          long long coff = n, roff = n;
          if (p.n_split > 0) {
            const int j = n / p.n_split, co = n % p.n_split;
            coff = (long long)j * p.c_split_stride + co;
            roff = (long long)j * p.r_split_stride + co;
          }
          if (rrow) {
            const float2 rr = *reinterpret_cast<const float2*>(rrow + roff);
            v.x += rr.x; v.y += rr.y;
          }
          if (crow2)
            *reinterpret_cast<float2*>(crow2 + coff) = make_float2(act_tc(v.x, p.act2), act_tc(v.y, p.act2));
          *reinterpret_cast<float2*>(crow + coff) = make_float2(act_tc(v.x, p.post_act), act_tc(v.y, p.post_act));
        }
      }
    }
  }
}

constexpr int RB_B_BYTES = 64 * 128;
constexpr int RB_STAGE_BYTES = TC_A_BYTES + 2 * RB_B_BYTES;
constexpr int RB_STAGES = 6;

struct RbParams {
  float* out;
  long long o_i_stride, o_o_stride;
  const float* b1;
  const float* b2;
  int I_out, i_tiles, m_tiles;
};

template <int C>
struct RbCfg {
  static constexpr int N1 = C / 2;
  static constexpr int KCH = C / 32;
  static constexpr int P1 = 3 * KCH;
  static constexpr int NS = C / 64;
  static constexpr int K2 = N1 / 32;
  static constexpr int H_BYTES = K2 * TC_A_BYTES;
  static constexpr int SMEM_BYTES = RB_STAGES * RB_STAGE_BYTES + H_BYTES + 1024  + 256 ;
  static constexpr bool ring_ok() {
    for (int j = 0; j < NS; ++j)
      for (int kc = 0; kc < KCH; ++kc)
        if ((P1 + j) % RB_STAGES == (2 * KCH + kc) % RB_STAGES) return false;
    return RB_STAGES >= KCH + NS;
  }
  static_assert(ring_ok(), "ring too small for the held residual stages");
  static_assert(K2 * 2 * RB_B_BYTES <= RB_STAGE_BYTES, "a phase-2 slice must fit one stage");
};

template <int C>
__global__ void __launch_bounds__(TC_THREADS, 1)
resblock_tc_kernel(const __grid_constant__ CUtensorMap tmY, const __grid_constant__ CUtensorMap tmW1,
                   const __grid_constant__ CUtensorMap tmW1lo, const __grid_constant__ CUtensorMap tmW2,
                   const __grid_constant__ CUtensorMap tmW2lo, const RbParams p) {
  using Cfg = RbCfg<C>;
  constexpr int S = RB_STAGES;
  constexpr int CH = TC_CHUNK_STAGES;
  constexpr int N1 = Cfg::N1, NR1 = N1 / 2, KCH = Cfg::KCH, P1 = Cfg::P1;
  extern __shared__ uint8_t smem_raw[];
  uint8_t* smem = smem_raw + ((1024u - (smem_u32(smem_raw) & 1023u)) & 1023u);
  uint8_t* hs = smem + S * RB_STAGE_BYTES;
  uint64_t* full = reinterpret_cast<uint64_t*>(hs + Cfg::H_BYTES);
  uint64_t* empty = full + S;
  const int warp = threadIdx.x / 32, lane = threadIdx.x % 32;

  if (threadIdx.x == 0) {
    for (int s = 0; s < S; ++s) {
      mbar_init(&full[s], 1);
      mbar_init(&empty[s], TC_CONSUMER_WARPS);
    }
    fence_barrier_init();
  }
  __syncthreads();

  if (warp == TC_CONSUMER_WARPS) {
    if (elect_one()) {
      tma_prefetch_desc(&tmY);
      tma_prefetch_desc(&tmW1);
      tma_prefetch_desc(&tmW1lo);
      tma_prefetch_desc(&tmW2);
      tma_prefetch_desc(&tmW2lo);
      int g = 0;
      for (int t = blockIdx.x; t < p.m_tiles; t += gridDim.x) {
        const int i0 = (t % p.i_tiles) * TC_BM, ot = t / p.i_tiles;
        for (int kit = 0; kit < P1; ++kit, ++g) {
          const int s = g % S;
          mbar_wait(&empty[s], ((g / S) & 1) ^ 1);
          const int tap = kit / KCH, kc = kit % KCH;
          uint8_t* st = smem + s * RB_STAGE_BYTES;
          mbar_arrive_expect_tx(&full[s], TC_A_BYTES + 2 * N1 * 128);
          tma_load_3d(st, &tmY, &full[s], kc * TC_BKE, i0, ot + tap);
          tma_load_2d(st + TC_A_BYTES, &tmW1, &full[s], kit * TC_BKE, 0);
          tma_load_2d(st + TC_A_BYTES + RB_B_BYTES, &tmW1lo, &full[s], kit * TC_BKE, 0);
        }
        for (int ns = 0; ns < Cfg::NS; ++ns, ++g) {
          const int s = g % S;
          mbar_wait(&empty[s], ((g / S) & 1) ^ 1);
          uint8_t* st = smem + s * RB_STAGE_BYTES;
          mbar_arrive_expect_tx(&full[s], Cfg::K2 * 2 * RB_B_BYTES);
#pragma unroll
          for (int kc = 0; kc < Cfg::K2; ++kc) {
            tma_load_2d(st + kc * 2 * RB_B_BYTES, &tmW2, &full[s], kc * TC_BKE, ns * 64);
            tma_load_2d(st + kc * 2 * RB_B_BYTES + RB_B_BYTES, &tmW2lo, &full[s], kc * TC_BKE, ns * 64);
          }
        }
      }
    }
    return;
  }

  const int wg = warp / 4, wq = warp % 4, gq = lane / 4, tq = lane % 4;
  const int r0 = wg * 64 + wq * 16 + gq;
  const uint32_t a_row = (uint32_t)r0 * 128u + (uint32_t)tq * 4u, a_sw = (uint32_t)(r0 & 7);
  const uint32_t smem0 = smem_u32(smem), hs0 = smem_u32(hs);
  int g = 0;
  for (int t = blockIdx.x; t < p.m_tiles; t += gridDim.x) {
    const int i0 = (t % p.i_tiles) * TC_BM, ot = t / p.i_tiles;
    const int g_res = g + 2 * KCH;
    {
      float acc[NR1], d0[NR1], d1[NR1];
#pragma unroll
      for (int j = 0; j < NR1; ++j) acc[j] = d0[j] = d1[j] = 0.f;
      for (int k0 = 0; k0 < P1; k0 += CH) {
        const int nst = P1 - k0 < CH ? P1 - k0 : CH;
        for (int u = 0; u < nst; ++u, ++g) {
          const int s = g % S;
          mbar_wait(&full[s], (g / S) & 1);
          const uint32_t st = smem0 + (uint32_t)(s * RB_STAGE_BYTES);
          uint32_t ah[4][4], al[4][4];
          tc_build_a<true, true>(st, a_row, a_sw, ah, al);
          wgmma_fence();
          tc_mma_stage<N1, true>(d0, d1, ah, al, gmma_desc_sw128(st + TC_A_BYTES), gmma_desc_sw128(st + TC_A_BYTES + RB_B_BYTES),
                                 u == 0);
          wgmma_commit();
          wgmma_wait<0>();
          __syncwarp();
          if (lane == 0 && k0 + u < 2 * KCH) mbar_arrive(&empty[s]);
        }
        fence_acc(d0);
        fence_acc(d1);
#pragma unroll
        for (int j = 0; j < NR1; ++j) acc[j] += d0[j] + d1[j];
      }
      named_bar_sync(1 + wg, 128);
#pragma unroll
      for (int hh = 0; hh < 2; ++hh) {
        const int r = r0 + 8 * hh;
#pragma unroll
        for (int b = 0; b < N1 / 8; ++b) {
          const int n = 8 * b + 2 * tq;
          const float2 bb = *reinterpret_cast<const float2*>(p.b1 + n);
          float2 v = make_float2(acc[4 * b + 2 * hh], acc[4 * b + 2 * hh + 1]);
          v.x += bb.x; v.y += bb.y;
          const uint32_t cc = (uint32_t)(n % 32);
          const uint32_t addr = hs0 + (uint32_t)(n / 32) * TC_A_BYTES + (uint32_t)r * 128u + (((cc >> 2) ^ (uint32_t)(r & 7)) << 4) +
                                (cc & 3u) * 4u;
          asm volatile("st.shared.v2.f32 [%0], {%1, %2};" ::"r"(addr), "f"(act_tc(v.x, ACT_ELU)), "f"(act_tc(v.y, ACT_ELU))
                       : "memory");
        }
      }
      named_bar_sync(1 + wg, 128);
    }
    for (int ns = 0; ns < Cfg::NS; ++ns, ++g) {
      const int s = g % S;
      mbar_wait(&full[s], (g / S) & 1);
      const uint32_t st = smem0 + (uint32_t)(s * RB_STAGE_BYTES);
      float acc[32], d0[32], d1[32];
#pragma unroll
      for (int j = 0; j < 32; ++j) d0[j] = d1[j] = 0.f;
#pragma unroll
      for (int kc = 0; kc < Cfg::K2; ++kc) {
        uint32_t ah[4][4], al[4][4];
        tc_build_a<true, false>(hs0 + (uint32_t)(kc * TC_A_BYTES), a_row, a_sw, ah, al);
        const uint32_t wst = st + (uint32_t)(kc * 2 * RB_B_BYTES);
        wgmma_fence();
        tc_mma_stage<64, true>(d0, d1, ah, al, gmma_desc_sw128(wst), gmma_desc_sw128(wst + RB_B_BYTES), kc == 0);
        wgmma_commit();
        wgmma_wait<0>();
      }
      __syncwarp();
      if (lane == 0) mbar_arrive(&empty[s]);
      fence_acc(d0);
      fence_acc(d1);
#pragma unroll
      for (int j = 0; j < 32; ++j) {
        acc[j] = 0.f;
        acc[j] += d0[j] + d1[j];
      }
#pragma unroll
      for (int hh = 0; hh < 2; ++hh) {
        const int r = r0 + 8 * hh;
        const int i = i0 + r;
        if (i >= p.I_out) continue;
        float* orow = p.out + (long long)ot * p.o_o_stride + (long long)i * p.o_i_stride;
#pragma unroll
        for (int b = 0; b < 8; ++b) {
          const int n = ns * 64 + 8 * b + 2 * tq;
          const float2 bb = *reinterpret_cast<const float2*>(p.b2 + n);
          float2 v = make_float2(acc[4 * b + 2 * hh], acc[4 * b + 2 * hh + 1]);
          v.x += bb.x; v.y += bb.y;
          const uint32_t cc = (uint32_t)(n % 32);
          const int rs = (g_res + n / 32) % S;
          const float2 rr = *reinterpret_cast<const float2*>(smem + rs * RB_STAGE_BYTES + r * 128 +
                                                             (((cc >> 2) ^ (uint32_t)(r & 7)) << 4) + (cc & 3u) * 4u);
          v.x += rr.x; v.y += rr.y;
          *reinterpret_cast<float2*>(orow + n) = make_float2(act_tc(v.x, ACT_ELU), act_tc(v.y, ACT_ELU));
        }
      }
      __syncwarp();
      if (lane == 0) {
        mbar_arrive(&empty[(g_res + 2 * ns) % S]);
        mbar_arrive(&empty[(g_res + 2 * ns + 1) % S]);
      }
    }
  }
}

typedef CUresult (*EncodeTiledFn)(CUtensorMap*, CUtensorMapDataType, cuuint32_t, void*, const cuuint64_t*, const cuuint64_t*,
                                  const cuuint32_t*, const cuuint32_t*, CUtensorMapInterleave, CUtensorMapSwizzle,
                                  CUtensorMapL2promotion, CUtensorMapFloatOOBfill);

static EncodeTiledFn get_encode_fn() {
  static EncodeTiledFn fn = nullptr;
  if (!fn) {
    void* p = nullptr;
    cudaDriverEntryPointQueryResult q;
    if (cudaGetDriverEntryPoint("cuTensorMapEncodeTiled", &p, cudaEnableDefault, &q) == cudaSuccess && p) fn = (EncodeTiledFn)p;
  }
  return fn;
}

}
using namespace rstnet;

struct rstnet_tc_plan {
  CUtensorMap tmA, tmW, tmWlo;
  TcParams p;
  dim3 grid;
  int bn, prec;
};

template <int BN, int PREC, bool PRE_ELU, bool KP>
static int tc_launch(const rstnet_tc_plan* pl, cudaStream_t st) {
  using Cfg = TcCfg<BN, PREC>;
  static unsigned long long attr = 0;
  smem_optin(gemm_tc_kernel<BN, PREC, PRE_ELU, KP>, Cfg::SMEM_BYTES, attr);
  gemm_tc_kernel<BN, PREC, PRE_ELU, KP><<<pl->grid, TC_THREADS, Cfg::SMEM_BYTES, st>>>(pl->tmA, pl->tmW, pl->tmWlo, pl->p);
  count_launch();
  return check_launch("gemm_tc");
}

template <int BN, int PREC>
static int tc_launch_mode(const rstnet_tc_plan* pl, cudaStream_t st) {
  const bool elu = pl->p.pre_act == ACT_ELU;
  if (pl->p.kpair) return elu ? tc_launch<BN, PREC, true, true>(pl, st) : tc_launch<BN, PREC, false, true>(pl, st);
  return elu ? tc_launch<BN, PREC, true, false>(pl, st) : tc_launch<BN, PREC, false, false>(pl, st);
}

extern "C" int rstnet_tc_gemm_create_ex(const rstnet_tc_gemm_desc* d, int32_t kpair, rstnet_tc_plan** out) {
  RSTNET_REQUIRE(d && out, "tc_gemm_create: null argument");
  RSTNET_REQUIRE(kpair >= -1 && kpair <= 1, "tc_gemm_create: kpair must be -1 (auto), 0 or 1 (got %d)", kpair);
  RSTNET_REQUIRE(d->A && d->W && d->C, "tc_gemm_create: null tensor pointer");
  RSTNET_REQUIRE(d->precision != 0 || d->W_lo, "tc_gemm_create: precision 0 (3xTF32) needs W_lo");
  RSTNET_REQUIRE(d->Kc > 0 && d->Kc % TC_BKE == 0, "tc_gemm_create: Kc (%d) must be a multiple of %d", d->Kc, TC_BKE);
  RSTNET_REQUIRE(d->N > 0 && d->N % 4 == 0, "tc_gemm_create: N (%d) must be a multiple of 4", d->N);
  RSTNET_REQUIRE(d->taps >= 1 && d->I_out > 0 && d->O_out > 0, "tc_gemm_create: bad shape");
  RSTNET_REQUIRE(d->precision == 0 || d->precision == 1, "tc_gemm_create: precision must be 0 (3xTF32) or 1 (TF32)");
  RSTNET_REQUIRE(d->pre_act == ACT_NONE || d->pre_act == ACT_ELU, "tc_gemm_create: pre_act must be NONE or ELU (got %d)", d->pre_act);
  RSTNET_REQUIRE((uintptr_t)d->A % 16 == 0 && (uintptr_t)d->W % 16 == 0 && (uintptr_t)d->C % 16 == 0 &&
                     d->a_i_stride % 4 == 0 && d->a_o_stride % 4 == 0 && d->c_i_stride % 4 == 0 && d->c_o_stride % 4 == 0 &&
                     d->c_split_stride % 4 == 0 && d->n_split % 4 == 0,
                 "tc_gemm_create: 16-byte alignment required");
  EncodeTiledFn enc = get_encode_fn();
  RSTNET_REQUIRE(enc != nullptr, "tc_gemm_create: cuTensorMapEncodeTiled unavailable (no CUDA driver?)");
  rstnet_tc_plan* pl = new rstnet_tc_plan();
  const int N = d->N;
  const int sms = sm_count();
  pl->bn = N >= 64 ? 64 : 32;
  const int i_tiles = ceil_div(d->I_out, TC_BM);
  {
    const long long mt = (long long)i_tiles * d->O_out;
    const long long t64 = mt * ceil_div(N, 64), t32 = mt * ceil_div(N, 32);
    if (pl->bn == 64 && ((t32 + sms - 1) / sms) * 2 <= ((t64 + sms - 1) / sms) * 3) pl->bn = 32;
  }
  pl->prec = d->precision;
  const int n_tiles = ceil_div(N, pl->bn);
  if (kpair < 0) {
    const long long total_k = (long long)d->taps * (d->Kc / TC_BKE);
    const long long t128 = (long long)i_tiles * d->O_out * n_tiles, t64 = (long long)ceil_div(d->I_out, TC_BM / 2) * d->O_out * n_tiles;
    const long long pair_k = (total_k + 2 * TC_CHUNK_STAGES - 1) / (2 * TC_CHUNK_STAGES) * TC_CHUNK_STAGES;
    kpair = t128 <= sms && ((t64 + sms - 1) / sms) * pair_k < total_k;
  }
  const int bm = kpair ? TC_BM / 2 : TC_BM;
  {
    cuuint64_t gdim[3] = {(cuuint64_t)d->a_c_extent, (cuuint64_t)d->a_i_extent, (cuuint64_t)d->a_o_extent};
    cuuint64_t gstr[2] = {(cuuint64_t)d->a_i_stride * 4, (cuuint64_t)d->a_o_stride * 4};
    cuuint32_t box[3] = {TC_BKE, (cuuint32_t)bm, 1};
    cuuint32_t estr[3] = {1, 1, 1};
    CUresult r = enc(&pl->tmA, CU_TENSOR_MAP_DATA_TYPE_FLOAT32, 3, (void*)d->A, gdim, gstr, box, estr, CU_TENSOR_MAP_INTERLEAVE_NONE,
                     CU_TENSOR_MAP_SWIZZLE_128B, CU_TENSOR_MAP_L2_PROMOTION_L2_128B, CU_TENSOR_MAP_FLOAT_OOB_FILL_NONE);
    if (r != CUDA_SUCCESS) {
      delete pl;
      set_error("tc_gemm_create: cuTensorMapEncodeTiled(A) failed with %d", (int)r);
      return 3;
    }
  }
  {
    cuuint64_t gdim[2] = {(cuuint64_t)d->taps * d->Kc, (cuuint64_t)N};
    cuuint64_t gstr[1] = {(cuuint64_t)d->taps * d->Kc * 4};
    cuuint32_t box[2] = {TC_BKE, (cuuint32_t)pl->bn};
    cuuint32_t estr[2] = {1, 1};
    CUresult r = enc(&pl->tmW, CU_TENSOR_MAP_DATA_TYPE_FLOAT32, 2, (void*)d->W, gdim, gstr, box, estr, CU_TENSOR_MAP_INTERLEAVE_NONE,
                     CU_TENSOR_MAP_SWIZZLE_128B, CU_TENSOR_MAP_L2_PROMOTION_L2_256B, CU_TENSOR_MAP_FLOAT_OOB_FILL_NONE);
    if (r == CUDA_SUCCESS && d->W_lo)
      r = enc(&pl->tmWlo, CU_TENSOR_MAP_DATA_TYPE_FLOAT32, 2, (void*)d->W_lo, gdim, gstr, box, estr, CU_TENSOR_MAP_INTERLEAVE_NONE,
              CU_TENSOR_MAP_SWIZZLE_128B, CU_TENSOR_MAP_L2_PROMOTION_L2_256B, CU_TENSOR_MAP_FLOAT_OOB_FILL_NONE);
    else
      pl->tmWlo = pl->tmW;
    if (r != CUDA_SUCCESS) {
      delete pl;
      set_error("tc_gemm_create: cuTensorMapEncodeTiled(W) failed with %d", (int)r);
      return 3;
    }
  }
  TcParams& p = pl->p;
  p.C2 = d->C2; p.act2 = d->act2;
  p.C = d->C; p.c_i_stride = d->c_i_stride; p.c_o_stride = d->c_o_stride; p.c_split_stride = d->c_split_stride;
  p.R = d->R; p.r_i_stride = d->r_i_stride; p.r_o_stride = d->r_o_stride; p.r_split_stride = d->r_split_stride;
  p.bias = d->bias; p.scale = d->scale; p.n_split = d->n_split;
  p.I_out = d->I_out; p.O_out = d->O_out; p.N = N; p.Kc = d->Kc;
  p.taps = d->taps; p.tap_di = d->tap_di; p.tap_do = d->tap_do; p.o_mul = d->o_mul; p.kchunks = d->Kc / TC_BKE;
  p.pre_act = d->pre_act; p.post_act = d->post_act;
  p.kpair = kpair;
  p.i_tiles = ceil_div(d->I_out, bm);
  p.m_tiles = p.i_tiles * d->O_out;
  p.n_tiles = n_tiles;
  const long long tiles = (long long)p.m_tiles * p.n_tiles;
  pl->grid = dim3((unsigned)(tiles < sms ? tiles : sms));
  *out = pl;
  return 0;
}

extern "C" int rstnet_tc_gemm_create(const rstnet_tc_gemm_desc* d, rstnet_tc_plan** out) {
  return rstnet_tc_gemm_create_ex(d, -1, out);
}

extern "C" int rstnet_tc_gemm_run(const rstnet_tc_plan* pl, rstnet_stream_t stream) {
  RSTNET_REQUIRE(pl != nullptr, "tc_gemm_run: null plan");
  cudaStream_t st = (cudaStream_t)stream;
  if (pl->prec == 0) return pl->bn == 64 ? tc_launch_mode<64, 0>(pl, st) : tc_launch_mode<32, 0>(pl, st);
  return pl->bn == 64 ? tc_launch_mode<64, 1>(pl, st) : tc_launch_mode<32, 1>(pl, st);
}

extern "C" void rstnet_tc_gemm_destroy(rstnet_tc_plan* pl) { delete pl; }

struct rstnet_tc_resblock_plan {
  CUtensorMap tmY, tmW1, tmW1lo, tmW2, tmW2lo;
  RbParams p;
  dim3 grid;
  int channels;
};

static int encode_2d(CUtensorMap* m, const float* base, int cols, int rows, int box_rows) {
  cuuint64_t gdim[2] = {(cuuint64_t)cols, (cuuint64_t)rows};
  cuuint64_t gstr[1] = {(cuuint64_t)cols * 4};
  cuuint32_t box[2] = {TC_BKE, (cuuint32_t)box_rows};
  cuuint32_t estr[2] = {1, 1};
  return (int)get_encode_fn()(m, CU_TENSOR_MAP_DATA_TYPE_FLOAT32, 2, (void*)base, gdim, gstr, box, estr, CU_TENSOR_MAP_INTERLEAVE_NONE,
                              CU_TENSOR_MAP_SWIZZLE_128B, CU_TENSOR_MAP_L2_PROMOTION_L2_256B, CU_TENSOR_MAP_FLOAT_OOB_FILL_NONE);
}

extern "C" int rstnet_tc_resblock_create(const rstnet_tc_resblock_desc* d, rstnet_tc_resblock_plan** out) {
  RSTNET_REQUIRE(d && out, "tc_resblock_create: null argument");
  RSTNET_REQUIRE(d->Y && d->W1 && d->W1_lo && d->b1 && d->W2 && d->W2_lo && d->b2 && d->out, "tc_resblock_create: null pointer");
  const int Cc = d->channels;
  RSTNET_REQUIRE(Cc == 64 || Cc == 128, "tc_resblock_create: channels must be 64 or 128 (got %d)", Cc);
  RSTNET_REQUIRE(d->I_out > 0 && d->O_out > 0 && d->y_rows >= d->O_out + 2, "tc_resblock_create: bad shape");
  RSTNET_REQUIRE((uintptr_t)d->Y % 16 == 0 && (uintptr_t)d->W1 % 16 == 0 && (uintptr_t)d->W1_lo % 16 == 0 && (uintptr_t)d->W2 % 16 == 0 &&
                     (uintptr_t)d->W2_lo % 16 == 0 && (uintptr_t)d->out % 16 == 0 && (uintptr_t)d->b1 % 8 == 0 &&
                     (uintptr_t)d->b2 % 8 == 0 && d->y_i_stride % 4 == 0 && d->y_o_stride % 4 == 0 && d->out_i_stride % 4 == 0 &&
                     d->out_o_stride % 4 == 0,
                 "tc_resblock_create: 16-byte alignment required");
  RSTNET_REQUIRE(get_encode_fn() != nullptr, "tc_resblock_create: cuTensorMapEncodeTiled unavailable (no CUDA driver?)");
  rstnet_tc_resblock_plan* pl = new rstnet_tc_resblock_plan();
  pl->channels = Cc;
  int r;
  {
    cuuint64_t gdim[3] = {(cuuint64_t)Cc, (cuuint64_t)d->I_out, (cuuint64_t)d->y_rows};
    cuuint64_t gstr[2] = {(cuuint64_t)d->y_i_stride * 4, (cuuint64_t)d->y_o_stride * 4};
    cuuint32_t box[3] = {TC_BKE, TC_BM, 1};
    cuuint32_t estr[3] = {1, 1, 1};
    r = (int)get_encode_fn()(&pl->tmY, CU_TENSOR_MAP_DATA_TYPE_FLOAT32, 3, (void*)d->Y, gdim, gstr, box, estr, CU_TENSOR_MAP_INTERLEAVE_NONE,
                             CU_TENSOR_MAP_SWIZZLE_128B, CU_TENSOR_MAP_L2_PROMOTION_L2_128B, CU_TENSOR_MAP_FLOAT_OOB_FILL_NONE);
  }
  if (r == CUDA_SUCCESS) r = encode_2d(&pl->tmW1, d->W1, 3 * Cc, Cc / 2, Cc / 2);
  if (r == CUDA_SUCCESS) r = encode_2d(&pl->tmW1lo, d->W1_lo, 3 * Cc, Cc / 2, Cc / 2);
  if (r == CUDA_SUCCESS) r = encode_2d(&pl->tmW2, d->W2, Cc / 2, Cc, 64);
  if (r == CUDA_SUCCESS) r = encode_2d(&pl->tmW2lo, d->W2_lo, Cc / 2, Cc, 64);
  if (r != CUDA_SUCCESS) {
    delete pl;
    set_error("tc_resblock_create: cuTensorMapEncodeTiled failed with %d", r);
    return 3;
  }
  RbParams& p = pl->p;
  p.out = d->out; p.o_i_stride = d->out_i_stride; p.o_o_stride = d->out_o_stride;
  p.b1 = d->b1; p.b2 = d->b2;
  p.I_out = d->I_out;
  p.i_tiles = ceil_div(d->I_out, TC_BM);
  p.m_tiles = p.i_tiles * d->O_out;
  const int sms = sm_count();
  pl->grid = dim3((unsigned)(p.m_tiles < sms ? p.m_tiles : sms));
  *out = pl;
  return 0;
}

template <int Cc>
static int rb_launch(const rstnet_tc_resblock_plan* pl, cudaStream_t st) {
  constexpr int smem = RbCfg<Cc>::SMEM_BYTES;
  static unsigned long long attr = 0;
  smem_optin(resblock_tc_kernel<Cc>, smem, attr);
  resblock_tc_kernel<Cc><<<pl->grid, TC_THREADS, smem, st>>>(pl->tmY, pl->tmW1, pl->tmW1lo, pl->tmW2, pl->tmW2lo, pl->p);
  count_launch();
  return check_launch("tc_resblock");
}

extern "C" int rstnet_tc_resblock_run(const rstnet_tc_resblock_plan* pl, rstnet_stream_t stream) {
  RSTNET_REQUIRE(pl != nullptr, "tc_resblock_run: null plan");
  cudaStream_t st = (cudaStream_t)stream;
  return pl->channels == 64 ? rb_launch<64>(pl, st) : rb_launch<128>(pl, st);
}

extern "C" void rstnet_tc_resblock_destroy(rstnet_tc_resblock_plan* pl) { delete pl; }
extern "C" int rstnet_tc_gemm_grid(const rstnet_tc_plan* pl, int32_t* gx, int32_t* gy, int32_t* bn) {
  if (!pl) return 1;
  *gx = ceil_div(pl->p.I_out, TC_BM) * pl->p.O_out; *gy = pl->p.n_tiles; *bn = pl->bn;
  return 0;
}
extern "C" int rstnet_tc_gemm_kpair(const rstnet_tc_plan* pl, int32_t* on) {
  if (!pl) return 1;
  *on = pl->p.kpair;
  return 0;
}

namespace rstnet {
__global__ void tf32_split_kernel(const float* __restrict__ x, float* __restrict__ hi, float* __restrict__ lo, long long n) {
  for (long long i = (long long)blockIdx.x * blockDim.x + threadIdx.x; i < n; i += (long long)gridDim.x * blockDim.x) {
    const float v = x[i], h = tf32_rna(v);
    hi[i] = h;
    lo[i] = tf32_rna_lo(v, h);
  }
}
}

extern "C" int rstnet_tf32_split_f32(const float* x, float* hi, float* lo, int64_t n, rstnet_stream_t stream) {
  RSTNET_REQUIRE(x && hi && lo, "tf32_split: null pointer");
  if (n <= 0) return 0;
  int g = ceil_div(n, 256);
  if (g > sm_count() * 8) g = sm_count() * 8;
  rstnet::tf32_split_kernel<<<g, 256, 0, (cudaStream_t)stream>>>(x, hi, lo, n);
  count_launch();
  return check_launch("tf32_split");
}
```

### rstnet_b200/ops.py

```python
from __future__ import annotations

import ctypes as C
import gc
from typing import Optional

import torch

from . import _lib
from ._lib import ACT_ELU, ACT_GELU, ACT_NONE, GemmRowsArgs, RowCopy, TcGemmDesc


def _stream() -> int:
    return torch.cuda.current_stream().cuda_stream


def capture(fn) -> torch.cuda.CUDAGraph:
    g = torch.cuda.CUDAGraph()
    enabled = gc.isenabled()
    gc.disable()
    try:
        with torch.cuda.graph(g):
            fn()
    finally:
        if enabled:
            gc.enable()
    return g


def _p(t: Optional[torch.Tensor]) -> Optional[int]:
    return None if t is None else t.data_ptr()


def _cuda(*ts):
    for t in ts:
        if t is not None and not t.is_cuda:
            raise _lib.RstnetError("rstnet_b200 ops need CUDA tensors (there is no CPU path)")


def gemm_rows(A: torch.Tensor, a_off: int, a_bs: int, a_rs: int, Wt: torch.Tensor, C_: torch.Tensor, c_off: int,
              c_bs: int, c_rs: int, batch: int, rows: int, *, bias=None, scale=None, R=None, r_off: int = 0,
              r_bs: int = 0, r_rs: int = 0, pre_act: int = ACT_NONE, post_act: int = ACT_NONE, taps: int = 1,
              tap_stride: int = 0) -> None:
    _cuda(A, Wt, C_, bias, scale, R)
    K, N = Wt.shape
    a = GemmRowsArgs()
    a.A = A.data_ptr() + 4 * a_off
    a.a_batch_stride, a.a_row_stride = a_bs, a_rs
    a.Wt = Wt.data_ptr()
    a.bias, a.scale = _p(bias), _p(scale)
    a.R = None if R is None else R.data_ptr() + 4 * r_off
    a.r_batch_stride, a.r_row_stride = r_bs, r_rs
    a.C = C_.data_ptr() + 4 * c_off
    a.c_batch_stride, a.c_row_stride = c_bs, c_rs
    a.batch, a.rows, a.N, a.K = batch, rows, N, K
    a.pre_act, a.post_act = pre_act, post_act
    a.taps, a.tap_stride = taps, tap_stride
    _lib.check(_lib.lib().rstnet_gemm_rows_f32(C.byref(a), _stream()), "gemm_rows_f32")


def tf32_split(w: torch.Tensor):
    _cuda(w)
    w = w.contiguous()
    both = torch.empty((2,) + tuple(w.shape), dtype=w.dtype, device=w.device)
    hi, lo = both[0], both[1]
    _lib.check(_lib.lib().rstnet_tf32_split_f32(w.data_ptr(), hi.data_ptr(), lo.data_ptr(), w.numel(), _stream()), "tf32_split")
    return hi, lo


class TcGemm:

    def __init__(self, A, a_off, a_i_stride, a_o_stride, a_c_extent, a_i_extent, a_o_extent, W, Kc, C_, c_off, c_i_stride,
                 c_o_stride, I_out, O_out, *, taps=1, tap_di=0, tap_do=0, o_mul=1, bias=None, scale=None, R=None, r_off=0,
                 r_i_stride=0, r_o_stride=0, n_split=0, c_split_stride=0, r_split_stride=0, pre_act=ACT_NONE,
                 post_act=ACT_NONE, precision=0, W_lo=None, C2=None, c2_off=0, act2=ACT_NONE):
        _cuda(A, W, C_, bias, scale, R, W_lo)
        N, Ktot = W.shape
        if precision == 0 and W_lo is None:
            W, W_lo = tf32_split(W)
        assert Ktot == taps * Kc, (Ktot, taps, Kc)
        d = TcGemmDesc()
        d.A = A.data_ptr() + 4 * a_off
        d.a_i_stride, d.a_o_stride = a_i_stride, a_o_stride
        d.a_c_extent, d.a_i_extent, d.a_o_extent = a_c_extent, a_i_extent, a_o_extent
        d.taps, d.tap_di, d.tap_do, d.o_mul = taps, tap_di, tap_do, o_mul
        d.W, d.W_lo, d.N, d.Kc, d.I_out, d.O_out = W.data_ptr(), _p(W_lo), N, Kc, I_out, O_out
        d.C = C_.data_ptr() + 4 * c_off
        d.c_i_stride, d.c_o_stride, d.c_split_stride = c_i_stride, c_o_stride, c_split_stride
        d.R = None if R is None else R.data_ptr() + 4 * r_off
        d.r_i_stride, d.r_o_stride, d.r_split_stride = r_i_stride, r_o_stride, r_split_stride
        d.bias, d.scale = _p(bias), _p(scale)
        d.n_split, d.pre_act, d.post_act, d.precision = n_split, pre_act, post_act, precision
        d.C2 = None if C2 is None else C2.data_ptr() + 4 * c2_off
        d.act2 = act2
        self._keep = (A, W, W_lo, C_, bias, scale, R, C2)
        self.flops = 2.0 * I_out * O_out * N * Ktot
        in_rows = min(a_o_extent, O_out * o_mul + (taps - 1) * max(tap_do, 0))
        n_out = I_out * O_out * N
        self.bytes = 4.0 * (a_c_extent * a_i_extent * in_rows + (2 if W_lo is not None else 1) * N * Ktot
                            + n_out * (2 if C2 is not None else 1) + (n_out if R is not None else 0))
        self._h = C.c_void_p()
        _lib.check(_lib.lib().rstnet_tc_gemm_create(C.byref(d), C.byref(self._h)), "tc_gemm_create")

    def run(self):
        _lib.check(_lib.lib().rstnet_tc_gemm_run(self._h, _stream()), "tc_gemm_run")

    def __del__(self):
        h = getattr(self, "_h", None)
        if h:
            try:
                _lib.lib().rstnet_tc_gemm_destroy(h)
            except Exception:
                pass
            self._h = None


class TcResblock:

    def __init__(self, Y, y_off, y_i_stride, y_o_stride, y_rows, I_out, O_out, W1, W1_lo, b1, W2, W2_lo, b2, out, out_off,
                 out_i_stride, out_o_stride):
        _cuda(Y, W1, W1_lo, b1, W2, W2_lo, b2, out)
        Cc = W2.shape[0]
        assert tuple(W1.shape) == (Cc // 2, 3 * Cc) and tuple(W2.shape) == (Cc, Cc // 2), (W1.shape, W2.shape)
        d = _lib.TcResblockDesc()
        d.Y = Y.data_ptr() + 4 * y_off
        d.y_i_stride, d.y_o_stride = y_i_stride, y_o_stride
        d.channels, d.I_out, d.O_out, d.y_rows = Cc, I_out, O_out, y_rows
        d.W1, d.W1_lo, d.b1 = W1.data_ptr(), W1_lo.data_ptr(), b1.data_ptr()
        d.W2, d.W2_lo, d.b2 = W2.data_ptr(), W2_lo.data_ptr(), b2.data_ptr()
        d.out = out.data_ptr() + 4 * out_off
        d.out_i_stride, d.out_o_stride = out_i_stride, out_o_stride
        self._keep = (Y, W1, W1_lo, b1, W2, W2_lo, b2, out)
        self.shape = dict(C=Cc, I=I_out, O=O_out)
        n = I_out * O_out
        self.flops = 2.0 * n * (W1.numel() + W2.numel())
        self.bytes = 4.0 * (Cc * I_out * (O_out + 2) + 2 * (W1.numel() + W2.numel()) + b1.numel() + b2.numel() + n * Cc)
        self._h = C.c_void_p()
        _lib.check(_lib.lib().rstnet_tc_resblock_create(C.byref(d), C.byref(self._h)), "tc_resblock_create")

    def run(self):
        _lib.check(_lib.lib().rstnet_tc_resblock_run(self._h, _stream()), "tc_resblock_run")

    def __del__(self):
        h = getattr(self, "_h", None)
        if h:
            try:
                _lib.lib().rstnet_tc_resblock_destroy(h)
            except Exception:
                pass
            self._h = None


def conv1d_cin1(x, x_bs, x_ts, w, bias, out, out_off, out_bs, out_ts, batch, T, Cout, k, post_act=ACT_NONE, out2=None,
                out2_off=0, act2=ACT_NONE):
    _cuda(x, w, out, out2)
    _lib.check(_lib.lib().rstnet_conv1d_cin1_f32(x.data_ptr(), x_bs, x_ts, w.data_ptr(), _p(bias), out.data_ptr() + 4 * out_off,
                                                 None if out2 is None else out2.data_ptr() + 4 * out2_off, out_bs, out_ts,
                                                 batch, T, Cout, k, post_act, act2, _stream()), "conv1d_cin1")


def conv1d_cout1(x, x_bs, x_ts, w, bias, out, out_bs, batch, T, Cin, k):
    _cuda(x, w, out)
    _lib.check(_lib.lib().rstnet_conv1d_cout1_f32(x.data_ptr(), x_bs, x_ts, w.data_ptr(), _p(bias), out.data_ptr(), out_bs,
                                                  batch, T, Cin, k, _stream()), "conv1d_cout1")


def convtr1d_depthwise(x, x_bs, x_ts, w, out, out_off, out_bs, out_ts, batch, T, Cch, stride):
    _cuda(x, w, out)
    _lib.check(_lib.lib().rstnet_convtr1d_depthwise_f32(x.data_ptr(), x_bs, x_ts, w.data_ptr(), out.data_ptr() + 4 * out_off,
                                                        out_bs, out_ts, batch, T, Cch, stride, _stream()), "convtr1d_depthwise")


def rows_fill(buf, bs, batch, Cch, row0, nrows, mode=0, src_row=0, only_if_zero=None, channels_per_stream=0):
    _cuda(buf)
    oz_stride = 1 if (only_if_zero is not None and only_if_zero.numel() > 1) else 0
    _lib.check(_lib.lib().rstnet_rows_fill_f32(buf.data_ptr(), bs, batch, Cch, row0, nrows, mode, src_row,
                                               _p(only_if_zero), oz_stride, channels_per_stream, _stream()), "rows_fill")


def rows_fill_tail(buf, bs, batch, Cch, row0, nrows, mode, valid, valid_div=1, channels_per_stream=0):
    _cuda(buf, valid)
    _lib.check(_lib.lib().rstnet_rows_fill_tail_f32(buf.data_ptr(), bs, batch, Cch, row0, nrows, mode, valid.data_ptr(), valid_div,
                                                    channels_per_stream, _stream()), "rows_fill_tail")


def rows_copy_table(table_dev: torch.Tensor, n_entries: int, batch: int, active: Optional[torch.Tensor] = None):
    _lib.check(_lib.lib().rstnet_rows_copy_table_f32(table_dev.data_ptr(), n_entries, batch, _p(active), _stream()), "rows_copy_table")


def make_copy_table(entries, device) -> torch.Tensor:
    arr = (RowCopy * len(entries))()
    for i, (t, bs, c, s, d, n, cps) in enumerate(entries):
        if n > 0 and not (s >= d):
            raise _lib.RstnetError("carry copy must move rows towards the front (src_row >= dst_row)")
        arr[i].buf, arr[i].batch_stride, arr[i].C, arr[i].src_row, arr[i].dst_row, arr[i].nrows = t.data_ptr(), bs, c, s, d, n
        arr[i].cps = cps
    raw = bytes(arr)
    return torch.frombuffer(bytearray(raw), dtype=torch.uint8).to(device)


def counter_add(counter: torch.Tensor, delta: int, active: Optional[torch.Tensor] = None):
    if active is not None and active.numel() != counter.numel():
        active = None
    _lib.check(_lib.lib().rstnet_counter_add(counter.data_ptr(), delta, counter.numel(), _p(active), _stream()), "counter_add")


def gen_rows_advance(tokens: torch.Tensor, rec: torch.Tensor, row_valid: torch.Tensor, status: torch.Tensor, card: int):
    B, dep_q = rec.shape[0], row_valid.shape[1]
    _lib.check(_lib.lib().rstnet_lm_gen_rows_advance(tokens.data_ptr(), tokens.stride(0), rec.data_ptr(), row_valid.data_ptr(),
                                                     row_valid.stride(0), status.data_ptr(), B, dep_q, card,
                                                     _stream()), "lm_gen_rows_advance")


def _ostride(offset: torch.Tensor) -> int:
    return 1 if offset.numel() > 1 else 0


def layer_norm(x, x_off, x_bs, w, b, y, batch, rows, dim, eps):
    _cuda(x, w, b, y)
    _lib.check(_lib.lib().rstnet_layer_norm_f32(x.data_ptr() + 4 * x_off, x_bs, w.data_ptr(), b.data_ptr(), y.data_ptr(),
                                                batch, rows, dim, eps, _stream()), "layer_norm")


def rope_kv_append(qkv, q_bs, q_ts, kv, offset, freqs, batch, T, H, D, cap):
    _cuda(qkv, kv, offset, freqs)
    _lib.check(_lib.lib().rstnet_rope_kv_append_f32(qkv.data_ptr(), q_bs, q_ts, kv.data_ptr(), offset.data_ptr(), _ostride(offset),
                                                    freqs.data_ptr(), batch, T, H, D, cap, _stream()), "rope_kv_append")


def rope_ring_attention(qkv, q_bs, q_ts, kv, offset, freqs, out, o_bs, o_ts, batch, T, H, D, cap, context):
    _cuda(qkv, kv, offset, freqs, out)
    _lib.check(_lib.lib().rstnet_rope_ring_attention_f32(qkv.data_ptr(), q_bs, q_ts, kv.data_ptr(), offset.data_ptr(), _ostride(offset),
                                                         freqs.data_ptr(), out.data_ptr(), o_bs, o_ts, batch, T, H, D, cap, context,
                                                         _stream()), "rope_ring_attention")


def ring_attention(qkv, q_bs, q_ts, kv, offset, out, o_bs, o_ts, batch, T, H, D, cap, context, linear):
    _cuda(qkv, kv, offset, out)
    _lib.check(_lib.lib().rstnet_ring_attention_f32(qkv.data_ptr(), q_bs, q_ts, kv.data_ptr(), offset.data_ptr(), _ostride(offset),
                                                    out.data_ptr(), o_bs, o_ts, batch, T, H, D, cap, context, int(linear),
                                                    _stream()), "ring_attention")


def rvq_encode_workspace(N, n_q, dim, bins) -> int:
    return int(_lib.lib().rstnet_rvq_encode_workspace(N, n_q, dim, bins))


def rvq_encode(x, ldx, E, Et, enorm, codes, work, N, T, n_q, ns, dim, bins, time_major=False):
    _cuda(x, E, Et, enorm, codes, work)
    _lib.check(_lib.lib().rstnet_rvq_encode_f32(x.data_ptr(), ldx, E.data_ptr(), Et.data_ptr(), enorm.data_ptr(),
                                                codes.data_ptr(), work.data_ptr(), N, T, n_q, ns, dim, bins, int(time_major),
                                                _stream()), "rvq_encode")


def rvq_decode_gather(codes, E, q, N, T, n_q, ns, dim, bins, time_major=False):
    _cuda(codes, E, q)
    _lib.check(_lib.lib().rstnet_rvq_decode_gather_f32(codes.data_ptr(), E.data_ptr(), q.data_ptr(), N, T, n_q, ns, dim,
                                                       bins, int(time_major), _stream()), "rvq_decode_gather")


def stft_loss_workspace(clips, max_len, hop) -> int:
    return int(_lib.lib().rstnet_stft_loss_workspace(clips, max_len, hop))


def stft_loss_sums(ref, deg, offsets, lengths, clips, min_len, max_len, n_fft, hop, win, twiddle, window, sums, n_res, res,
                   ws):
    _cuda(ref, deg, offsets, lengths, twiddle, window, sums, ws)
    _lib.check(_lib.lib().rstnet_stft_loss_sums_f32(ref.data_ptr(), deg.data_ptr(), offsets.data_ptr(), lengths.data_ptr(),
                                                    clips, min_len, max_len, n_fft, hop, win, twiddle.data_ptr(),
                                                    window.data_ptr(), sums.data_ptr(), n_res, res, ws.data_ptr(),
                                                    ws.numel() * ws.element_size(), _stream()), "stft_loss_sums")


def sisnr_moments_workspace(clips, max_len) -> int:
    return int(_lib.lib().rstnet_sisnr_moments_workspace(clips, max_len))


def sisnr_moments(ref, deg, offsets, lengths, clips, max_len, moments, ws):
    _cuda(ref, deg, offsets, lengths, moments, ws)
    _lib.check(_lib.lib().rstnet_sisnr_moments_f32(ref.data_ptr(), deg.data_ptr(), offsets.data_ptr(), lengths.data_ptr(),
                                                   clips, max_len, moments.data_ptr(), ws.data_ptr(),
                                                   ws.numel() * ws.element_size(), _stream()), "sisnr_moments")
```

Before: 44690.

## Add split-K with workspace reduction to the tensor-core GEMM

Adds a split-K mode to the persistent TMA tensor-core GEMM. Each output tile's K chunks are divided among several CTAs, which write partial sums to a global workspace, and the last arriving CTA (found via an atomic counter) reduces them before the epilogue. A cost model picks the split factor automatically when tiles are too few to fill the SMs, and codec plans share one workspace. This trades extra global partial-sum traffic and a counter sync for better SM occupancy on small-M, deep-K GEMMs.

```diff
diff --git a/include/rstnet_b200.h b/include/rstnet_b200.h
--- a/include/rstnet_b200.h
+++ b/include/rstnet_b200.h
@@ -60,6 +60,10 @@
 int rstnet_tc_gemm_grid(const rstnet_tc_plan* plan, int32_t* grid_x, int32_t* grid_y, int32_t* tile_n);
 int rstnet_tc_gemm_create_ex(const rstnet_tc_gemm_desc* desc, int32_t kpair, rstnet_tc_plan** out);
 int rstnet_tc_gemm_kpair(const rstnet_tc_plan* plan, int32_t* on);
+int rstnet_tc_gemm_create_split(const rstnet_tc_gemm_desc* desc, int32_t kpair, int32_t ksplit, rstnet_tc_plan** out);
+int rstnet_tc_gemm_ksplit(const rstnet_tc_plan* plan, int32_t* ksplit);
+int64_t rstnet_tc_gemm_workspace_bytes(const rstnet_tc_gemm_desc* desc, int32_t kpair, int32_t ksplit);
+int rstnet_tc_gemm_set_workspace(rstnet_tc_plan* plan, void* workspace, int64_t bytes);
 typedef struct rstnet_tc_resblock_plan rstnet_tc_resblock_plan;
 typedef struct {
   const float* Y;
diff --git a/rstnet_b200/_lib.py b/rstnet_b200/_lib.py
--- a/rstnet_b200/_lib.py
+++ b/rstnet_b200/_lib.py
@@ -11,7 +11,8 @@
 SYMBOLS = [
     "rstnet_version", "rstnet_last_error", "rstnet_launch_count", "rstnet_device_error_flags",
     "rstnet_gemm_rows_f32", "rstnet_tc_gemm_create", "rstnet_tc_gemm_run", "rstnet_tc_gemm_destroy", "rstnet_tc_gemm_grid",
-    "rstnet_tc_gemm_create_ex", "rstnet_tc_gemm_kpair",
+    "rstnet_tc_gemm_create_ex", "rstnet_tc_gemm_kpair", "rstnet_tc_gemm_create_split", "rstnet_tc_gemm_ksplit",
+    "rstnet_tc_gemm_workspace_bytes", "rstnet_tc_gemm_set_workspace",
     "rstnet_tc_resblock_create", "rstnet_tc_resblock_run", "rstnet_tc_resblock_destroy", "rstnet_tf32_split_f32", "rstnet_conv1d_cin1_f32", "rstnet_conv1d_cout1_f32",
     "rstnet_convtr1d_depthwise_f32", "rstnet_rows_fill_f32", "rstnet_rows_copy_table_f32",
     "rstnet_counter_add", "rstnet_layer_norm_f32", "rstnet_rope_kv_append_f32",
@@ -120,6 +121,11 @@
     L.rstnet_tc_gemm_grid.argtypes = [vp, C.POINTER(i32), C.POINTER(i32), C.POINTER(i32)]
     L.rstnet_tc_gemm_create_ex.argtypes = [C.POINTER(TcGemmDesc), i32, C.POINTER(C.c_void_p)]
     L.rstnet_tc_gemm_kpair.argtypes = [vp, C.POINTER(i32)]
+    L.rstnet_tc_gemm_create_split.argtypes = [C.POINTER(TcGemmDesc), i32, i32, C.POINTER(C.c_void_p)]
+    L.rstnet_tc_gemm_ksplit.argtypes = [vp, C.POINTER(i32)]
+    L.rstnet_tc_gemm_workspace_bytes.argtypes = [C.POINTER(TcGemmDesc), i32, i32]
+    L.rstnet_tc_gemm_workspace_bytes.restype = i64
+    L.rstnet_tc_gemm_set_workspace.argtypes = [vp, vp, i64]
     L.rstnet_tc_resblock_create.argtypes = [C.POINTER(TcResblockDesc), C.POINTER(C.c_void_p)]
     L.rstnet_tc_resblock_run.argtypes = [vp, vp]
     L.rstnet_tc_resblock_destroy.argtypes = [vp]
diff --git a/rstnet_b200/codec.py b/rstnet_b200/codec.py
--- a/rstnet_b200/codec.py
+++ b/rstnet_b200/codec.py
@@ -490,6 +490,7 @@
         self.ops_list = []
         self.graph: Optional[torch.cuda.CUDAGraph] = None
         self.precision = eng.m.decoder_precision if isinstance(self, _DecPlan) else eng.m.tc_precision
+        self.ws = ops.TcWorkspace(eng.device)
 
     def buf(self, ctx, T, extra, C) -> _Buf:
         return _Buf(self.B, ctx, T, extra, C, self.eng.device, self.tc)
@@ -560,7 +561,7 @@
             kw.update(C2=out2.t, c2_off=out2.off(out2_row0), act2=ACT_ELU)
         w_hi, w_lo = self.tc_weights(pack)
         plan = ops.TcGemm(A.t, A.off(a_row0), Cin, B * Cin, Cin, B, A.rows - a_row0, w_hi, Cin, out.t, out.off(out_row0),
-                          out.C, (tr_stride or 1) * B * out.C, B, T_out, W_lo=w_lo, **kw)
+                          out.C, (tr_stride or 1) * B * out.C, B, T_out, W_lo=w_lo, workspace=self.ws, **kw)
         self.add(plan.run)
 
     def linear(self, A_t, a_rows_view, K, pack, out_t, out_view, N_row_stride, *, post=ACT_NONE, scale=None, R_view=None):
@@ -578,7 +579,7 @@
             kw.update(R=out_t, r_off=R_view[0], r_i_stride=N_row_stride, r_o_stride=rpb * N_row_stride)
         w_hi, w_lo = self.tc_weights(pack)
         plan = ops.TcGemm(A_t, a_off, K, rpb * K, K, rpb, 1, w_hi, K, out_t, c_off, N_row_stride, rpb * N_row_stride, rpb, 1,
-                          W_lo=w_lo, **kw)
+                          W_lo=w_lo, workspace=self.ws, **kw)
         self.add(plan.run)
 
     def rows_view(self, X: _Buf, row0: int, nrows: int):
@@ -737,6 +738,7 @@
         self.add(lambda: ops.rvq_encode(xproj, 2 * cd, eng.E, eng.Et, eng.enorm, codes, work, B * T5, T5, m.n_q, m.n_q_semantic,
                                         cd, m.codebook_size, time_major=self.tc))
         self.finish_streaming([xin] + ya + r_ + [y4, X], F)
+        self.ws.bind()
 
     def tail_fill(self, X: _Buf, T: int, mode: int, valid: torch.Tensor, div: int):
         bs, nb, C = (0, 1, self.B * X.C) if self.tc else (X.bs, self.B, X.C)
@@ -814,6 +816,7 @@
                                           m.last_kernel_size))
         self.finish_streaming([qup, X] + a + yda, F)
         self.debug_bufs = {"qup": [qup], "X": [X], "a": a, "yd": yd, "yda": yda, "hd": [b for b in hd_ if b is not None]}
+        self.ws.bind()
 
     def run(self, codes: torch.Tensor, graphs: Optional[bool]) -> torch.Tensor:
         self.codes_in.copy_(codes)
diff --git a/rstnet_b200/csrc/gemm_tc.cu b/rstnet_b200/csrc/gemm_tc.cu
--- a/rstnet_b200/csrc/gemm_tc.cu
+++ b/rstnet_b200/csrc/gemm_tc.cu
@@ -30,6 +30,10 @@
   int pre_act, post_act, i_tiles;
   int m_tiles, n_tiles;
   int kpair;
+  int ksplit;
+  int ws_slots;
+  int* counters;
+  float* partials;
 };
 
 template <int BN, int PREC>
@@ -41,6 +45,7 @@
   static constexpr int SMEM_BYTES = STAGES * STAGE_BYTES + 1024  + 256 ;
   static constexpr int Q_PIECES = BN / 32;
   static_assert(STAGES % 2 == 0 && 2 * Q_PIECES <= STAGES, "K-pair rings and queue");
+  static_assert(STAGES * 8 * 2 + 4 * 8 + 4 <= 256, "barriers and the split-K flag fit the barrier area");
 };
 
 __device__ __forceinline__ float tf32_rna(float x) {
@@ -98,7 +103,7 @@
   }
 }
 
-template <int BN, int PREC, bool PRE_ELU, bool KP>
+template <int BN, int PREC, bool PRE_ELU, bool KP, bool SK>
 __global__ void __launch_bounds__(TC_THREADS, 1)
 gemm_tc_kernel(const __grid_constant__ CUtensorMap tmA, const __grid_constant__ CUtensorMap tmW,
                const __grid_constant__ CUtensorMap tmWlo, const TcParams p) {
@@ -112,9 +117,12 @@
   uint64_t* empty = full + S;
   uint64_t* qfull = empty + S;
   uint64_t* qempty = qfull + 2;
+  int* last_flag = reinterpret_cast<int*>(qempty + 2);
   const int warp = threadIdx.x / 32, lane = threadIdx.x % 32;
   const int total_k = p.taps * p.kchunks;
-  const int total_tiles = p.m_tiles * p.n_tiles;
+  const int nch = (total_k + TC_CHUNK_STAGES - 1) / TC_CHUNK_STAGES;
+  const int nsplit = SK ? p.ksplit : 1;
+  const int total_units = p.m_tiles * p.n_tiles * nsplit;
   const int bm = KP ? TC_BM / 2 : TC_BM;
   const int R = KP ? S / 2 : S;
 
@@ -137,11 +145,14 @@
       tma_prefetch_desc(&tmW);
       if (Cfg::SPLIT) tma_prefetch_desc(&tmWlo);
       int pos0 = 0, ph0 = 0, pos1 = 0, ph1 = 0;
-      for (int t = blockIdx.x; t < total_tiles; t += gridDim.x) {
+      for (int u = blockIdx.x; u < total_units; u += gridDim.x) {
+        const int t = u / nsplit, sp = u % nsplit;
         const int nt = t % p.n_tiles, mt = t / p.n_tiles;
         const int i0 = (mt % p.i_tiles) * bm, ot = mt / p.i_tiles, n0 = nt * BN;
-        for (int kit = 0; kit < total_k; ++kit) {
-          const int w = KP ? (kit / TC_CHUNK_STAGES) & 1 : 0;
+        const int cb = sp * nch / nsplit, ce = (sp + 1) * nch / nsplit;
+        const int kend = ce * TC_CHUNK_STAGES < total_k ? ce * TC_CHUNK_STAGES : total_k;
+        for (int kit = cb * TC_CHUNK_STAGES; kit < kend; ++kit) {
+          const int w = KP ? (kit / TC_CHUNK_STAGES - cb) & 1 : 0;
           const int pos = w ? pos1 : pos0, ph = w ? ph1 : ph0;
           const int s = w * R + pos;
           const int npos = pos + 1 == R ? 0 : pos + 1, nph = ph ^ (npos == 0);
@@ -166,7 +177,6 @@
   float acc[NR], d0[NR], d1[NR];
 #pragma unroll
   for (int j = 0; j < NR; ++j) d0[j] = d1[j] = 0.f;
-  const int nch = (total_k + CH - 1) / CH;
   const bool sender = KP && wg == 1;
   auto qel = [&](int q, int j) {
     return reinterpret_cast<float*>(smem + (q * Cfg::Q_PIECES + j / 16) * Cfg::STAGE_BYTES + TC_A_BYTES / 2) +
@@ -181,13 +191,21 @@
     ++qn;
   };
   const int base = KP ? wg * R : 0;
+  const int sl_threads = KP ? 128 : 256, sl_tid = KP ? (threadIdx.x & 127) : threadIdx.x;
+  auto slot4 = [&](int t, int slot, int v) {
+    return reinterpret_cast<float4*>(p.partials + ((long long)t * p.ws_slots + slot) * (bm * BN)) + v * sl_threads + sl_tid;
+  };
+  const int c1 = nch / nsplit;
   int pos = 0, ph = 0;
-  for (int t = blockIdx.x; t < total_tiles; t += gridDim.x) {
+  for (int u = blockIdx.x; u < total_units; u += gridDim.x) {
+    const int t = u / nsplit, sp = u % nsplit;
     const int nt = t % p.n_tiles, mt = t / p.n_tiles;
     const int i0 = (mt % p.i_tiles) * bm, ot = mt / p.i_tiles, n0 = nt * BN;
+    const int cb = sp * nch / nsplit, ce = (sp + 1) * nch / nsplit;
+    const bool stash = SK && sp > 0;
 #pragma unroll
     for (int j = 0; j < NR; ++j) acc[j] = 0.f;
-    for (int c = KP ? wg : 0; c < nch; c += KP ? 2 : 1) {
+    for (int c = cb + (KP ? wg : 0); c < ce; c += KP ? 2 : 1) {
       const int k0 = c * CH;
       const int nst = total_k - k0 < CH ? total_k - k0 : CH;
       for (int u = 0; u < nst; ++u) {
@@ -209,19 +227,59 @@
       }
       fence_acc(d0);
       if (Cfg::SPLIT) fence_acc(d1);
-      if (sender) {
+      if (stash) {
+#pragma unroll
+        for (int v = 0; v < NR / 4; ++v) {
+          float4 q;
+          q.x = Cfg::SPLIT ? d0[4 * v] + d1[4 * v] : d0[4 * v];
+          q.y = Cfg::SPLIT ? d0[4 * v + 1] + d1[4 * v + 1] : d0[4 * v + 1];
+          q.z = Cfg::SPLIT ? d0[4 * v + 2] + d1[4 * v + 2] : d0[4 * v + 2];
+          q.w = Cfg::SPLIT ? d0[4 * v + 3] + d1[4 * v + 3] : d0[4 * v + 3];
+          __stcg(slot4(t, 1 + c - c1, v), q);
+        }
+      } else if (sender) {
         mbar_wait(&qempty[qn & 1], ((qn >> 1) & 1) ^ 1);
 #pragma unroll
         for (int j = 0; j < NR; ++j) *qel(qn & 1, j) = Cfg::SPLIT ? d0[j] + d1[j] : d0[j];
         mbar_arrive(&qfull[qn & 1]);
         ++qn;
       } else {
-        if (KP && c > 0) take_queued();
+        if (KP && c > cb) take_queued();
 #pragma unroll
         for (int j = 0; j < NR; ++j) acc[j] += Cfg::SPLIT ? d0[j] + d1[j] : d0[j];
       }
     }
-    if (KP && !sender && nch % 2 == 0) take_queued();
+    if (KP && !sender && !stash && (ce - cb) % 2 == 0) take_queued();
+    if (SK) {
+      if (sp == 0 && !sender) {
+#pragma unroll
+        for (int v = 0; v < NR / 4; ++v) __stcg(slot4(t, 0, v), make_float4(acc[4 * v], acc[4 * v + 1], acc[4 * v + 2], acc[4 * v + 3]));
+      }
+      __threadfence();
+      named_bar_sync(1, TC_CONSUMER_WARPS * 32);
+      if (threadIdx.x == 0) {
+        const int last = atomicAdd(&p.counters[t], 1) == nsplit - 1;
+        if (last) atomicExch(&p.counters[t], 0);
+        __threadfence();
+        *last_flag = last;
+      }
+      named_bar_sync(1, TC_CONSUMER_WARPS * 32);
+      if (!*last_flag || sender) continue;
+      if (sp != 0) {
+#pragma unroll
+        for (int v = 0; v < NR / 4; ++v) {
+          const float4 q = __ldcg(slot4(t, 0, v));
+          acc[4 * v] = q.x; acc[4 * v + 1] = q.y; acc[4 * v + 2] = q.z; acc[4 * v + 3] = q.w;
+        }
+      }
+      for (int c = c1; c < nch; ++c) {
+#pragma unroll
+        for (int v = 0; v < NR / 4; ++v) {
+          const float4 q = __ldcg(slot4(t, 1 + c - c1, v));
+          acc[4 * v] += q.x; acc[4 * v + 1] += q.y; acc[4 * v + 2] += q.z; acc[4 * v + 3] += q.w;
+        }
+      }
+    }
     if (sender) continue;
 #pragma unroll
     for (int h = 0; h < 2; ++h) {
@@ -483,33 +541,100 @@
   TcParams p;
   dim3 grid;
   int bn, prec;
+  long long ws_bytes;
 };
 
-template <int BN, int PREC, bool PRE_ELU, bool KP>
+template <int BN, int PREC, bool PRE_ELU, bool KP, bool SK>
 static int tc_launch(const rstnet_tc_plan* pl, cudaStream_t st) {
   using Cfg = TcCfg<BN, PREC>;
   static unsigned long long attr = 0;
-  smem_optin(gemm_tc_kernel<BN, PREC, PRE_ELU, KP>, Cfg::SMEM_BYTES, attr);
-  gemm_tc_kernel<BN, PREC, PRE_ELU, KP><<<pl->grid, TC_THREADS, Cfg::SMEM_BYTES, st>>>(pl->tmA, pl->tmW, pl->tmWlo, pl->p);
+  smem_optin(gemm_tc_kernel<BN, PREC, PRE_ELU, KP, SK>, Cfg::SMEM_BYTES, attr);
+  gemm_tc_kernel<BN, PREC, PRE_ELU, KP, SK><<<pl->grid, TC_THREADS, Cfg::SMEM_BYTES, st>>>(pl->tmA, pl->tmW, pl->tmWlo, pl->p);
   count_launch();
   return check_launch("gemm_tc");
 }
 
+template <int BN, int PREC, bool KP, bool SK>
+static int tc_launch_act(const rstnet_tc_plan* pl, cudaStream_t st) {
+  return pl->p.pre_act == ACT_ELU ? tc_launch<BN, PREC, true, KP, SK>(pl, st) : tc_launch<BN, PREC, false, KP, SK>(pl, st);
+}
+
 template <int BN, int PREC>
 static int tc_launch_mode(const rstnet_tc_plan* pl, cudaStream_t st) {
-  const bool elu = pl->p.pre_act == ACT_ELU;
-  if (pl->p.kpair) return elu ? tc_launch<BN, PREC, true, true>(pl, st) : tc_launch<BN, PREC, false, true>(pl, st);
-  return elu ? tc_launch<BN, PREC, true, false>(pl, st) : tc_launch<BN, PREC, false, false>(pl, st);
-}
-
-extern "C" int rstnet_tc_gemm_create_ex(const rstnet_tc_gemm_desc* d, int32_t kpair, rstnet_tc_plan** out) {
+  if (pl->p.ksplit > 1) return pl->p.kpair ? tc_launch_act<BN, PREC, true, true>(pl, st) : tc_launch_act<BN, PREC, false, true>(pl, st);
+  return pl->p.kpair ? tc_launch_act<BN, PREC, true, false>(pl, st) : tc_launch_act<BN, PREC, false, false>(pl, st);
+}
+
+struct TcGeom {
+  int bn, kpair, ksplit, bm, n_tiles, nch, slots;
+  long long tiles, ws_bytes;
+};
+
+constexpr long long TC_SPLIT_WS_CAP = 32ll << 20;
+constexpr int TC_SPLIT_MAX = 8;
+constexpr int TC_SPLIT_MIN_CHUNKS = 4;
+
+static long long tc_split_ws_bytes(long long tiles, int slots, int bm, int bn) {
+  return (tiles * 4 + 255) / 256 * 256 + tiles * slots * (long long)bm * bn * 4;
+}
+
+static void tc_geometry(const rstnet_tc_gemm_desc* d, int kpair, int ksplit, int sms, TcGeom* g) {
+  const int N = d->N;
+  g->bn = N >= 64 ? 64 : 32;
+  const int i_tiles = ceil_div(d->I_out, TC_BM);
+  {
+    const long long mt = (long long)i_tiles * d->O_out;
+    const long long t64 = mt * ceil_div(N, 64), t32 = mt * ceil_div(N, 32);
+    if (g->bn == 64 && ((t32 + sms - 1) / sms) * 2 <= ((t64 + sms - 1) / sms) * 3) g->bn = 32;
+  }
+  g->n_tiles = ceil_div(N, g->bn);
+  const long long total_k = (long long)d->taps * (d->Kc / TC_BKE);
+  g->nch = (int)((total_k + TC_CHUNK_STAGES - 1) / TC_CHUNK_STAGES);
+  if (kpair < 0) {
+    const long long t128 = (long long)i_tiles * d->O_out * g->n_tiles, t64 = (long long)ceil_div(d->I_out, TC_BM / 2) * d->O_out * g->n_tiles;
+    const long long pair_k = (total_k + 2 * TC_CHUNK_STAGES - 1) / (2 * TC_CHUNK_STAGES) * TC_CHUNK_STAGES;
+    kpair = t128 <= sms && ((t64 + sms - 1) / sms) * pair_k < total_k;
+  }
+  g->kpair = kpair;
+  g->bm = kpair ? TC_BM / 2 : TC_BM;
+  g->tiles = (long long)ceil_div(d->I_out, g->bm) * d->O_out * g->n_tiles;
+  if (ksplit < 0) {
+    const long long chunk_in = TC_CHUNK_STAGES * ((long long)g->bm * 128 + (long long)g->bn * 128 * (d->precision == 0 ? 2 : 1));
+    const long long slot = (long long)g->bm * g->bn * 4;
+    auto cost = [&](int s) {
+      const long long rounds = (g->tiles * s + sms - 1) / sms, per = (g->nch + s - 1) / s;
+      return rounds * per * (chunk_in + (s > 1 ? slot : 0)) + (s > 1 ? (long long)(g->nch - g->nch / s + 1) * slot : 0);
+    };
+    ksplit = 1;
+    long long best = cost(1) * 7 / 8;
+    for (int s = 2; s <= TC_SPLIT_MAX && g->nch / s >= TC_SPLIT_MIN_CHUNKS && g->tiles * s <= sms; ++s) {
+      if (tc_split_ws_bytes(g->tiles, g->nch - g->nch / s + 1, g->bm, g->bn) > TC_SPLIT_WS_CAP) break;
+      if (cost(s) < best) { best = cost(s); ksplit = s; }
+    }
+  }
+  g->ksplit = ksplit;
+  g->slots = ksplit > 1 ? g->nch - g->nch / ksplit + 1 : 0;
+  g->ws_bytes = ksplit > 1 ? tc_split_ws_bytes(g->tiles, g->slots, g->bm, g->bn) : 0;
+}
+
+static int tc_check_args(const rstnet_tc_gemm_desc* d, int32_t kpair, int32_t ksplit) {
+  RSTNET_REQUIRE(d, "tc_gemm_create: null argument");
+  RSTNET_REQUIRE(kpair >= -1 && kpair <= 1, "tc_gemm_create: kpair must be -1 (auto), 0 or 1 (got %d)", kpair);
+  RSTNET_REQUIRE(ksplit == -1 || ksplit >= 1, "tc_gemm_create: ksplit must be -1 (auto) or >= 1 (got %d)", ksplit);
+  RSTNET_REQUIRE(d->Kc > 0 && d->Kc % TC_BKE == 0, "tc_gemm_create: Kc (%d) must be a multiple of %d", d->Kc, TC_BKE);
+  RSTNET_REQUIRE(d->taps >= 1 && d->I_out > 0 && d->O_out > 0, "tc_gemm_create: bad shape");
+  const long long nch = ((long long)d->taps * (d->Kc / TC_BKE) + TC_CHUNK_STAGES - 1) / TC_CHUNK_STAGES;
+  RSTNET_REQUIRE(ksplit <= nch, "tc_gemm_create: ksplit (%d) exceeds the %lld promotion chunks of K", ksplit, nch);
+  return 0;
+}
+
+extern "C" int rstnet_tc_gemm_create_split(const rstnet_tc_gemm_desc* d, int32_t kpair, int32_t ksplit, rstnet_tc_plan** out) {
   RSTNET_REQUIRE(d && out, "tc_gemm_create: null argument");
-  RSTNET_REQUIRE(kpair >= -1 && kpair <= 1, "tc_gemm_create: kpair must be -1 (auto), 0 or 1 (got %d)", kpair);
+  *out = nullptr;
+  if (int rc = tc_check_args(d, kpair, ksplit)) return rc;
   RSTNET_REQUIRE(d->A && d->W && d->C, "tc_gemm_create: null tensor pointer");
   RSTNET_REQUIRE(d->precision != 0 || d->W_lo, "tc_gemm_create: precision 0 (3xTF32) needs W_lo");
-  RSTNET_REQUIRE(d->Kc > 0 && d->Kc % TC_BKE == 0, "tc_gemm_create: Kc (%d) must be a multiple of %d", d->Kc, TC_BKE);
   RSTNET_REQUIRE(d->N > 0 && d->N % 4 == 0, "tc_gemm_create: N (%d) must be a multiple of 4", d->N);
-  RSTNET_REQUIRE(d->taps >= 1 && d->I_out > 0 && d->O_out > 0, "tc_gemm_create: bad shape");
   RSTNET_REQUIRE(d->precision == 0 || d->precision == 1, "tc_gemm_create: precision must be 0 (3xTF32) or 1 (TF32)");
   RSTNET_REQUIRE(d->pre_act == ACT_NONE || d->pre_act == ACT_ELU, "tc_gemm_create: pre_act must be NONE or ELU (got %d)", d->pre_act);
   RSTNET_REQUIRE((uintptr_t)d->A % 16 == 0 && (uintptr_t)d->W % 16 == 0 && (uintptr_t)d->C % 16 == 0 &&
@@ -518,25 +643,15 @@
                  "tc_gemm_create: 16-byte alignment required");
   EncodeTiledFn enc = get_encode_fn();
   RSTNET_REQUIRE(enc != nullptr, "tc_gemm_create: cuTensorMapEncodeTiled unavailable (no CUDA driver?)");
-  rstnet_tc_plan* pl = new rstnet_tc_plan();
   const int N = d->N;
   const int sms = sm_count();
-  pl->bn = N >= 64 ? 64 : 32;
-  const int i_tiles = ceil_div(d->I_out, TC_BM);
-  {
-    const long long mt = (long long)i_tiles * d->O_out;
-    const long long t64 = mt * ceil_div(N, 64), t32 = mt * ceil_div(N, 32);
-    if (pl->bn == 64 && ((t32 + sms - 1) / sms) * 2 <= ((t64 + sms - 1) / sms) * 3) pl->bn = 32;
-  }
+  TcGeom g;
+  tc_geometry(d, kpair, ksplit, sms, &g);
+  rstnet_tc_plan* pl = new rstnet_tc_plan();
+  pl->bn = g.bn;
   pl->prec = d->precision;
-  const int n_tiles = ceil_div(N, pl->bn);
-  if (kpair < 0) {
-    const long long total_k = (long long)d->taps * (d->Kc / TC_BKE);
-    const long long t128 = (long long)i_tiles * d->O_out * n_tiles, t64 = (long long)ceil_div(d->I_out, TC_BM / 2) * d->O_out * n_tiles;
-    const long long pair_k = (total_k + 2 * TC_CHUNK_STAGES - 1) / (2 * TC_CHUNK_STAGES) * TC_CHUNK_STAGES;
-    kpair = t128 <= sms && ((t64 + sms - 1) / sms) * pair_k < total_k;
-  }
-  const int bm = kpair ? TC_BM / 2 : TC_BM;
+  pl->ws_bytes = g.ws_bytes;
+  const int bm = g.bm;
   {
     cuuint64_t gdim[3] = {(cuuint64_t)d->a_c_extent, (cuuint64_t)d->a_i_extent, (cuuint64_t)d->a_o_extent};
     cuuint64_t gstr[2] = {(cuuint64_t)d->a_i_stride * 4, (cuuint64_t)d->a_o_stride * 4};
@@ -576,22 +691,50 @@
   p.I_out = d->I_out; p.O_out = d->O_out; p.N = N; p.Kc = d->Kc;
   p.taps = d->taps; p.tap_di = d->tap_di; p.tap_do = d->tap_do; p.o_mul = d->o_mul; p.kchunks = d->Kc / TC_BKE;
   p.pre_act = d->pre_act; p.post_act = d->post_act;
-  p.kpair = kpair;
+  p.kpair = g.kpair;
+  p.ksplit = g.ksplit;
+  p.ws_slots = g.slots;
+  p.counters = nullptr;
+  p.partials = nullptr;
   p.i_tiles = ceil_div(d->I_out, bm);
   p.m_tiles = p.i_tiles * d->O_out;
-  p.n_tiles = n_tiles;
-  const long long tiles = (long long)p.m_tiles * p.n_tiles;
-  pl->grid = dim3((unsigned)(tiles < sms ? tiles : sms));
+  p.n_tiles = g.n_tiles;
+  const long long units = g.tiles * g.ksplit;
+  pl->grid = dim3((unsigned)(units < sms ? units : sms));
   *out = pl;
   return 0;
 }
 
+extern "C" int rstnet_tc_gemm_create_ex(const rstnet_tc_gemm_desc* d, int32_t kpair, rstnet_tc_plan** out) {
+  return rstnet_tc_gemm_create_split(d, kpair, 1, out);
+}
+
 extern "C" int rstnet_tc_gemm_create(const rstnet_tc_gemm_desc* d, rstnet_tc_plan** out) {
-  return rstnet_tc_gemm_create_ex(d, -1, out);
+  return rstnet_tc_gemm_create_split(d, -1, 1, out);
+}
+
+extern "C" int64_t rstnet_tc_gemm_workspace_bytes(const rstnet_tc_gemm_desc* d, int32_t kpair, int32_t ksplit) {
+  if (tc_check_args(d, kpair, ksplit)) return -1;
+  TcGeom g;
+  tc_geometry(d, kpair, ksplit, sm_count(), &g);
+  return g.ws_bytes;
+}
+
+extern "C" int rstnet_tc_gemm_set_workspace(rstnet_tc_plan* pl, void* ws, int64_t bytes) {
+  RSTNET_REQUIRE(pl != nullptr, "tc_gemm_set_workspace: null plan");
+  if (pl->p.ksplit == 1) return 0;
+  RSTNET_REQUIRE(ws != nullptr && bytes >= pl->ws_bytes,
+                 "tc_gemm_set_workspace: split-K plan needs %lld workspace bytes (got %lld)", pl->ws_bytes, (long long)bytes);
+  RSTNET_REQUIRE((uintptr_t)ws % 256 == 0, "tc_gemm_set_workspace: workspace must be 256-byte aligned");
+  const long long tiles = (long long)pl->p.m_tiles * pl->p.n_tiles;
+  pl->p.counters = reinterpret_cast<int*>(ws);
+  pl->p.partials = reinterpret_cast<float*>(reinterpret_cast<char*>(ws) + (tiles * 4 + 255) / 256 * 256);
+  return 0;
 }
 
 extern "C" int rstnet_tc_gemm_run(const rstnet_tc_plan* pl, rstnet_stream_t stream) {
   RSTNET_REQUIRE(pl != nullptr, "tc_gemm_run: null plan");
+  RSTNET_REQUIRE(pl->p.ksplit == 1 || pl->p.counters, "tc_gemm_run: split-K plan has no workspace (rstnet_tc_gemm_set_workspace)");
   cudaStream_t st = (cudaStream_t)stream;
   if (pl->prec == 0) return pl->bn == 64 ? tc_launch_mode<64, 0>(pl, st) : tc_launch_mode<32, 0>(pl, st);
   return pl->bn == 64 ? tc_launch_mode<64, 1>(pl, st) : tc_launch_mode<32, 1>(pl, st);
@@ -686,6 +829,11 @@
   *on = pl->p.kpair;
   return 0;
 }
+extern "C" int rstnet_tc_gemm_ksplit(const rstnet_tc_plan* pl, int32_t* ksplit) {
+  if (!pl) return 1;
+  *ksplit = pl->p.ksplit;
+  return 0;
+}
 
 namespace rstnet {
 __global__ void tf32_split_kernel(const float* __restrict__ x, float* __restrict__ hi, float* __restrict__ lo, long long n) {
diff --git a/rstnet_b200/ops.py b/rstnet_b200/ops.py
--- a/rstnet_b200/ops.py
+++ b/rstnet_b200/ops.py
@@ -67,12 +67,33 @@
     return hi, lo
 
 
+class TcWorkspace:
+
+    def __init__(self, device):
+        self.device, self.plans, self.t = device, [], None
+
+    def add(self, plan: "TcGemm"):
+        assert self.t is None, "TcWorkspace: plan added after bind()"
+        self.plans.append(plan)
+
+    @property
+    def nbytes(self) -> int:
+        return max((p.ws_bytes for p in self.plans), default=0)
+
+    def bind(self):
+        if self.nbytes:
+            self.t = torch.zeros(self.nbytes, dtype=torch.uint8, device=self.device)
+            for p in self.plans:
+                p.set_workspace(self.t)
+
+
 class TcGemm:
 
     def __init__(self, A, a_off, a_i_stride, a_o_stride, a_c_extent, a_i_extent, a_o_extent, W, Kc, C_, c_off, c_i_stride,
                  c_o_stride, I_out, O_out, *, taps=1, tap_di=0, tap_do=0, o_mul=1, bias=None, scale=None, R=None, r_off=0,
                  r_i_stride=0, r_o_stride=0, n_split=0, c_split_stride=0, r_split_stride=0, pre_act=ACT_NONE,
-                 post_act=ACT_NONE, precision=0, W_lo=None, C2=None, c2_off=0, act2=ACT_NONE):
+                 post_act=ACT_NONE, precision=0, W_lo=None, C2=None, c2_off=0, act2=ACT_NONE, kpair=-1, ksplit=-1,
+                 workspace: Optional[TcWorkspace] = None):
         _cuda(A, W, C_, bias, scale, R, W_lo)
         N, Ktot = W.shape
         if precision == 0 and W_lo is None:
@@ -99,7 +120,25 @@
         self.bytes = 4.0 * (a_c_extent * a_i_extent * in_rows + (2 if W_lo is not None else 1) * N * Ktot
                             + n_out * (2 if C2 is not None else 1) + (n_out if R is not None else 0))
         self._h = C.c_void_p()
-        _lib.check(_lib.lib().rstnet_tc_gemm_create(C.byref(d), C.byref(self._h)), "tc_gemm_create")
+        L = _lib.lib()
+        _lib.check(L.rstnet_tc_gemm_create_split(C.byref(d), kpair, ksplit, C.byref(self._h)), "tc_gemm_create_split")
+        self.desc = d
+        kp, ks = C.c_int32(), C.c_int32()
+        L.rstnet_tc_gemm_kpair(self._h, C.byref(kp))
+        L.rstnet_tc_gemm_ksplit(self._h, C.byref(ks))
+        self.kpair, self.ksplit = kp.value, ks.value
+        self.ws_bytes = int(L.rstnet_tc_gemm_workspace_bytes(C.byref(d), self.kpair, self.ksplit))
+        self._ws = None
+        if self.ws_bytes:
+            if workspace is None:
+                self.set_workspace(torch.zeros(self.ws_bytes, dtype=torch.uint8, device=C_.device))
+            else:
+                workspace.add(self)
+
+    def set_workspace(self, t: torch.Tensor):
+        _lib.check(_lib.lib().rstnet_tc_gemm_set_workspace(self._h, t.data_ptr(), t.numel() * t.element_size()),
+                   "tc_gemm_set_workspace")
+        self._ws = t
 
     def run(self):
         _lib.check(_lib.lib().rstnet_tc_gemm_run(self._h, _stream()), "tc_gemm_run")
```

Result: no change. 44930 (median of 6 runs) (+0.5%).
